# AgentMaker/PAPC

Measured on AMD Instinct MI355X. Metric: point-clouds/sec (fwd+bwd) PointNet++SSG B=32 N=4096, higher is better.
Workload: dtype f32

## Files before the change

### include/papc_hip.h

```cpp
#ifndef PAPC_HIP_H
#define PAPC_HIP_H

#include <stddef.h>
#include <stdint.h>

#ifdef __cplusplus
extern "C" {
#endif

#define PAPC_OK 0
#define PAPC_E_INVALID (-1)
#define PAPC_E_UNSUPPORTED (-2)
#define PAPC_E_LAUNCH (-3)

typedef void *papc_stream_t;

int papc_version(void);
#define PAPC_ABI_VERSION 8
int papc_abi_version(void);
int64_t papc_abi_sizeof(const char *struct_name);
const char *papc_last_error_string(void);


int papc_fps_f32(const float *xyz, int64_t sb, int64_t sn, int64_t sc, int B, int N, int npoint,
// ... 174 lines not shown
int papc_fold_jobs_f32(const papc_fold_job *jobs, int count, papc_stream_t stream);

#define PAPC_SA_MAX_LAYERS 8
#define PAPC_SA_IN_GROUP 0
#define PAPC_SA_IN_ROWS 1
#define PAPC_SA_NO_LINGATHER 1u
#define PAPC_SA_NO_XYZ1 2u
#define PAPC_SA_NO_NOSTORE 4u
#define PAPC_SA_NO_GMAX 8u
#define PAPC_SA_NO_FUSED_RED 16u
#define PAPC_SA_NO_COMPACT 32u
#define PAPC_SA_NO_PLANES 64u
#define PAPC_SA_NO_PLANES_POINTWISE 128u
#define PAPC_SA_NO_XYZ_FUSE 256u
#define PAPC_SA_NO_PSEL 1024u
#define PAPC_SA_NO_GSIGN 2048u
#define PAPC_SA_NO_WSTATS 512u
typedef struct papc_sa_desc {
    int32_t B, N, S, K, D;
    int32_t n_layers;
    int32_t cin;
    int32_t cout[PAPC_SA_MAX_LAYERS];
    int32_t input;
    int32_t identity_rows;
    int32_t xyz_first, pool, eval_bn, cut_gather_grad;
    float eps, momentum;
    uint32_t disable;
    int32_t inference;
    int32_t want_input_grad;
} papc_sa_desc;
typedef struct papc_sa_layer {
    const float *w, *b, *gamma, *beta;
    float *running_mean, *running_var;
} papc_sa_layer;
typedef struct papc_compact_src {
    const int32_t *start, *rows, *cidx, *seg_grp;
    const float *wrow, *coef;
    int32_t G;
} papc_compact_src;
typedef struct papc_sa_io {
    const float *xyz; int64_t sb, sn, sc;
    const float *new_xyz;
    const float *feats;
    const int32_t *idx;
    const float *x_rows;
    const float *xc; const double *xc_gram;
    const papc_compact_src *compact;
    const float *consts3; int32_t consts3_ld;
    papc_sa_layer layer[PAPC_SA_MAX_LAYERS];
    float *out;
    void *saved, *scratch;
    const papc_point_lists *plists;
    const float *wfeat;
} papc_sa_io;
typedef struct papc_sa_plan {
    papc_sa_desc d;
    int32_t cin0;
    int32_t lin0, xyz1, gmax, nostore, compact, sparse_max, planes;
    int64_t saved_bytes, fwd_scratch_bytes, bwd_scratch_bytes;
    int64_t off_y[PAPC_SA_MAX_LAYERS], off_cst[PAPC_SA_MAX_LAYERS], off_argmax;
} papc_sa_plan;
typedef struct papc_sa_grads {
    const float *gout;
    float *dw[PAPC_SA_MAX_LAYERS], *db[PAPC_SA_MAX_LAYERS], *dgamma[PAPC_SA_MAX_LAYERS], *dbeta[PAPC_SA_MAX_LAYERS];
    int32_t acc_w[PAPC_SA_MAX_LAYERS], acc_gb[PAPC_SA_MAX_LAYERS];
    const float *wt[PAPC_SA_MAX_LAYERS];
    float *grad_feats, *grad_x;
    struct papc_fold_list *defer;
} papc_sa_grads;
int papc_sa_mlp_plan(const papc_sa_desc *desc, const papc_sa_io *io, papc_sa_plan *plan);
int papc_sa_mlp_fwd(const papc_sa_plan *plan, const papc_sa_io *io, papc_stream_t stream);
int papc_sa_mlp_bwd(const papc_sa_plan *plan, const papc_sa_io *io, const papc_sa_grads *grads, papc_stream_t stream);

typedef struct papc_pfn_desc {
    int32_t P, T, C;
    float vx, vy, x_offset, y_offset;
    float eps, momentum;
    int32_t training;
    int32_t zero_padded;
} papc_pfn_desc;
typedef struct papc_pfn_io {
    const float *features; const int32_t *num_voxels, *coors;
    const float *w, *gamma, *beta;
    float *running_mean, *running_var;
    float *out;
    void *saved, *scratch;
    uint32_t *tickets;
} papc_pfn_io;
int papc_pfn_workspace(const papc_pfn_desc *desc, int64_t *saved_bytes, int64_t *scratch_bytes);
int papc_pfn_fwd(const papc_pfn_desc *desc, const papc_pfn_io *io, papc_stream_t stream);
int papc_pfn_bwd(const papc_pfn_desc *desc, const papc_pfn_io *io, const float *gout, float *dw, float *dgamma, float *dbeta, int accumulate,
                 papc_stream_t stream);


int papc_pfn_decorate_f32(const float *features, const int32_t *num_voxels, const int32_t *coors, int P, int T,
                          float vx, float vy, float x_offset, float y_offset, int with_distance, float *out,
                          papc_stream_t stream);
int papc_pfn_decorate_nf_f32(const float *features, int F, const int32_t *num_voxels, const int32_t *coors, int P, int T,
                             float vx, float vy, float x_offset, float y_offset, int with_distance, float *out, papc_stream_t stream);
int papc_pfn_stats_f32(const float *features, const int32_t *num_voxels, const int32_t *coors, int P, int T,
                       float vx, float vy, float x_offset, float y_offset, const float *w, int C,
                       float *stats_partial, int *n_blocks_out, papc_stream_t stream);
int papc_pfn_apply_f32(const float *features, const int32_t *num_voxels, const int32_t *coors, int P, int T,
                       float vx, float vy, float x_offset, float y_offset, const float *w, int C,
                       const float *scale, const float *shift, float *out, int32_t *argmax,
                       papc_stream_t stream);
// ... 156 lines not shown
typedef struct papc_pg_prep {
    int mode;
    int64_t M; int C;
    const float *x; int64_t ldx;
    const float *xyz; int64_t sb, sn, sc; const float *feats; int N, D, xyz_first;
    const float *dz;
    const float *gout, *ysel; const int32_t *argmax; int K;
    const float *stats; int parts;
    const float *gamma, *beta; float eps, momentum; float *running_mean, *running_var;
    float *mean, *invstd, *scale, *shift;
    const float *red; int red_parts;
    float *dgamma, *dbeta; int accumulate;
    void *planes, *planes_t;
} papc_pg_prep;
int papc_pg_prep_rows_f32(const papc_pg_prep *args, papc_stream_t stream);

#define PAPC_PG_STORE 0
#define PAPC_PG_FWD 1
#define PAPC_PG_FWD_GMAX 2
#define PAPC_PG_RED 3
typedef struct papc_pg_gemm {
    int epi;
    const void *a, *b;
    int R1, R2, K;
    float *c; int64_t ldc;
    int split; int64_t split_stride;
    const float *bias;
    float *stats;
    float *gmax, *gmin; int32_t *amax, *amin;
    const float *y_prev, *mean, *invstd, *scale, *shift;
    int family;
} papc_pg_gemm;
int papc_pg_gemm_f32(const papc_pg_gemm *args, papc_stream_t stream);
int papc_pg_gemm_group_f32(const papc_pg_gemm *args, int count, papc_stream_t stream);

int papc_pg_final_f32(const float *stats, int parts, int64_t M, int C, const float *gamma, const float *beta, float eps, float momentum,
                      float *mean, float *invstd, float *scale, float *shift, float *running_mean, float *running_var, float *gmax,
                      const float *gmin, const int32_t *amax, const int32_t *amin, int64_t G, float *out, int32_t *argmax, papc_stream_t stream);
int papc_pg_final_groups_f32(const float *stats, int parts, int64_t M, int C, const float *gamma, const float *beta, float eps, float momentum,
                             float *mean, float *invstd, float *scale, float *shift, float *running_mean, float *running_var, const float *gmax,
                             const float *gmin, const int32_t *amax, const int32_t *amin, int64_t G, int tiles_per_group, float *out, int32_t *argmax,
                             float *ysel, papc_stream_t stream);

typedef struct papc_pg_fold_job {
    const float *partial; int nsplit; int64_t stride, n;
    float *out; int accumulate;
} papc_pg_fold_job;
int papc_pg_fold_f32(const papc_pg_fold_job *jobs, int count, papc_stream_t stream);

int papc_transpose_batch_f32(const float *const *src, float *const *dst, const int *rows, const int *cols, int count, papc_stream_t stream);
int papc_transpose_batch_ld_f32(const float *const *src, const int *src_ld, float *const *dst, const int *rows, const int *cols, const int *copy, int count,
                                papc_stream_t stream);

int papc_fill_f32(float *p, int64_t n, float value, papc_stream_t stream);
int papc_copy2d_f32(const float *src, int64_t src_ld, float *dst, int64_t dst_ld, int rows, int cols, int transpose,
                    papc_stream_t stream);
int papc_reduce_partials_strided_f32(const float *partial, int n_chunks, int64_t ld, int rows, int cols, float *out,
                                     int64_t out_ld, int accumulate, papc_stream_t stream);
typedef struct papc_copy_job {
    const float *src;
    float *dst;
    int32_t B, R, C;
    int64_t sb, sr, sc, db, dr, dc;
} papc_copy_job;
int papc_copy_strided_batch_f32(const papc_copy_job *jobs, int count, papc_stream_t stream);
int papc_scale_by_f32(const float *x, const float *scalar, int64_t n, float *out, papc_stream_t stream);

int papc_adam_step_f32(float *param, const float *grad, float *exp_avg, float *exp_avg_sq, int64_t n,
                       float lr, double beta1, double beta2, float eps, float weight_decay, int step,
                       float grad_scale, papc_stream_t stream);
int papc_adam_step_zero_f32(float *param, float *grad, float *exp_avg, float *exp_avg_sq, int64_t n,
                            float lr, double beta1, double beta2, float eps, float weight_decay, int step,
                            float grad_scale, papc_stream_t stream);
int papc_adam_tick(int64_t *step_dev, papc_stream_t stream);
int papc_flag_set(uint32_t *flag, uint32_t value, int64_t *counter, papc_stream_t stream);
int papc_flag_wait(uint32_t *flag, int64_t max_spins, papc_stream_t stream);
int papc_flag_wait_slot(uint32_t *flag, int slot, int64_t max_spins, papc_stream_t stream);
int papc_adam_step_dev_f32(float *param, float *grad, float *exp_avg, float *exp_avg_sq, int64_t n, float lr, double beta1, double beta2,
                           float eps, float weight_decay, const int64_t *step_dev, float grad_scale, int zero_grad, papc_stream_t stream);

#define PAPC_K_FPS 0
#define PAPC_K_BALL_QUERY 1
#define PAPC_K_GROUP 2
#define PAPC_K_MLP_GEMM 3
#define PAPC_K_BN_RELU_MAX 4
#define PAPC_K_BWD_REDUCE 5
#define PAPC_K_BWD_DX 6
#define PAPC_K_BWD_DW 7
#define PAPC_K_PFN 8
#define PAPC_K_MISC 9
#define PAPC_K_COUNT 10
int papc_prof_enable(unsigned mask);
int papc_prof_reset(void);
int papc_prof_read(int kernel, double *total_ms, int64_t *launches);

int papc_knob_set(const char *name, int value);
int papc_knob_get(const char *name, int *value);

#ifdef __cplusplus
}
#endif
#endif
```

### papc_amd/_lib.py

```python
import ctypes
import os

_HERE = os.path.dirname(os.path.abspath(__file__))
LIB_PATH = os.environ.get("PAPC_LIB") or os.path.join(_HERE, "libpapc_hip.so")

ABI_VERSION = 8

c_p = ctypes.c_void_p
c_i = ctypes.c_int
c_l = ctypes.c_int64
c_f = ctypes.c_float


class PapcError(RuntimeError):
    pass


class GroupSrc(ctypes.Structure):
    _fields_ = [("xyz", c_p), ("sb", c_l), ("sn", c_l), ("sc", c_l), ("new_xyz", c_p), ("feats", c_p),
                ("idx", c_p), ("N", c_i), ("S", c_i), ("K", c_i), ("D", c_i), ("xyz_first", c_i),
                ("cidx", c_p), ("seg_grp", c_p), ("rows_dev", c_p), ("wstat", c_p), ("plists", c_p)]


class PointLists(ctypes.Structure):
# ... 93 lines not shown
    "papc_points_to_voxel_f32": (c_i, [c_p, c_i, c_i, c_p, c_p, c_i, c_i, c_i, c_p, c_p, c_p, c_p, c_p, ctypes.c_size_t, c_p]),
    "papc_pillar_scatter_f32": (c_i, [c_p, c_p, c_i, c_i, c_i, c_i, c_i, c_p, c_p, c_p]),
    "papc_pillar_scatter_bwd_f32": (c_i, [c_p, c_p, c_p, c_i, c_i, c_i, c_i, c_i, c_p, c_p]),
    "papc_head_fc_f32": (c_i, [c_p, c_p, c_p, c_p, c_p, c_i, c_i, c_i, c_i, c_f, c_f, c_p, c_p, c_p, c_f, c_p, c_i, c_p, c_p, c_p, c_p,
                               c_p, c_p, c_p]),
    "papc_head_bwd_f32": (c_i, [c_p, c_p, c_i, c_p, c_p, c_p, c_p, c_p, c_f, c_i, c_p, c_i, c_i, c_i, c_p, c_p, c_p, c_p, c_p, c_i, c_p]),
    "papc_softmax_xent_f32": (c_i, [c_p, c_p, c_i, c_i, c_p, c_p, c_p]),
    "papc_head_chain_fwd_f32": (c_i, [c_p, c_i, c_i, c_p, c_p, c_p, c_p, c_p, c_p, c_p]),
    "papc_head_chain_bwd_f32": (c_i, [c_p, c_i, c_i, c_p, c_p]),
    "papc_cloud_transform_f32": (c_i, [c_p, c_l, c_l, c_l, c_p, c_l, c_i, c_i, c_i, c_p, c_p]),
    "papc_cloud_transform_bwd_workspace": (ctypes.c_size_t, [c_i, c_i, c_i]),
    "papc_cloud_transform_bwd_f32": (c_i, [c_p, c_l, c_l, c_l, c_p, c_l, c_p, c_i, c_i, c_i, c_p, c_l, c_l, c_l, c_i, c_p, c_p, ctypes.c_size_t, c_p]),
    "papc_cloud_concat_conv_parts": (c_i, [c_i, c_i]),
    "papc_cloud_concat_conv_f32": (c_i, [c_p, c_l, c_p, c_p, c_p, c_i, c_i, c_i, c_i, c_i, c_p, c_p, c_p, c_p]),
    "papc_cloud_concat_conv_bwd_workspace": (ctypes.c_size_t, [c_i, c_i, c_i, c_i, c_i]),
    "papc_cloud_concat_conv_bwd_f32": (c_i, [c_p, c_p, c_p, c_p, c_p, c_p, c_p, c_p, c_p, c_l, c_p, c_p, c_i, c_i, c_i, c_i, c_i, c_p, c_l, c_i, c_p, c_p,
                                             c_p, c_p, c_p, ctypes.c_size_t, c_p]),
    "papc_nms_workspace": (ctypes.c_size_t, [c_i]),
    "papc_nms_f32": (c_i, [c_p, c_i, c_f, c_p, c_p, c_p, ctypes.c_size_t, c_p]),
    "papc_lingather_parts": (c_i, [c_l]),
    "papc_lingather_fwd_f32": (c_i, [c_p, c_p, c_i, c_p, c_i, c_i, c_p, c_i, c_p, c_p, c_p]),
    "papc_lingather_bwd_f32": (c_i, [c_p, c_p, c_i, c_i, c_p, c_p, c_p]),
    "papc_lingather_bwd_pp_f32": (c_i, [c_p, c_p, c_i, c_i, c_p, c_p, c_i, c_i, c_p, c_p, c_p, c_p]),
    "papc_lingather_list_parts": (c_i, [c_l]),
    "papc_lingather_bwd_parts": (c_i, [c_p, c_i, c_i]),
    "papc_lingather_bwd_lists_ok": (c_i, [c_p, c_i]),
    "papc_point_lists_f32": (c_i, [c_p, c_i, c_p, c_p, c_p, c_p, c_p, c_p]),
    "papc_lingather_bwd_pp_ok": (c_i, [c_p, c_i, c_i]),
    "papc_bn_max_prep_f32": (c_i, [c_p] * 10 + [c_l, c_i, c_i] + [c_p] * 6),
    "papc_mlp_max_nostore_ok": (c_i, [c_l, c_i, c_i, c_i]),
    "papc_mlp_bwd_dw_max_ws_floats": (c_l, [c_l, c_i, c_i]),
    "papc_mlp_bwd_dw_max_f32": (c_i, [c_p, c_p, c_i, c_p, c_p, c_p, c_p, c_p, c_p, c_p, c_l, c_i, c_i, c_p, c_p, c_i, c_p]),
    "papc_mlp_bwd_dx_xyz_ok": (c_i, [c_l, c_i, c_i]),
    "papc_mlp_bwd_dx_xyz_f32": (c_i, [c_p, c_p, c_l, c_i, c_i, c_p, c_p, c_p, c_p]),
    "papc_mlp_bwd_dx_max_f32": (c_i, [c_p, c_p, c_i, c_p, c_l, c_p, c_p, c_p, c_p, c_l, c_i, c_i, c_p, c_p, c_p]),
    "papc_mlp_xyz_ok": (c_i, [c_l, c_i, c_i]),
    "papc_xyz_parts": (c_i, [c_l]),
    "papc_xyz_bwd_parts": (c_i, [c_l]),
    "papc_xyz_group_f32": (c_i, [c_p, c_i, c_p, c_p, c_p]),
    "papc_xyz_gram_fold_f32": (c_i, [c_p, c_i, c_p, c_p]),
    "papc_xyz_l1_finalize_f32": (c_i, [c_p, c_i, c_l, c_p, c_i, c_i, c_p, c_p, c_p, c_f, c_f, c_i] + [c_p] * 9),
    "papc_xyz_l1_bwd_f32": (c_i, [c_p, c_p, c_p, c_l, c_i, c_p, c_p]),
    "papc_xyz_l1_bwd_finalize_f32": (c_i, [c_p, c_i, c_l, c_i, c_p, c_p, c_i, c_i] + [c_p] * 7 + [c_i, c_p]),
    "papc_pg_planes_bytes": (ctypes.c_size_t, [c_l, c_l]),
    "papc_pg_prep_weights_f32": (c_i, [c_p, c_i, c_p]),
    "papc_pg_prep_rows_f32": (c_i, [c_p, c_p]),
    "papc_pg_gemm_f32": (c_i, [c_p, c_p]),
    "papc_pg_gemm_group_f32": (c_i, [c_p, c_i, c_p]),
    "papc_pg_final_f32": (c_i, [c_p, c_i, c_l, c_i, c_p, c_p, c_f, c_f] + [c_p] * 10 + [c_l, c_p, c_p, c_p]),
    "papc_pg_final_groups_f32": (c_i, [c_p, c_i, c_l, c_i, c_p, c_p, c_f, c_f] + [c_p] * 10 + [c_l, c_i, c_p, c_p, c_p, c_p]),
    "papc_pg_fold_f32": (c_i, [c_p, c_i, c_p]),
    "papc_transpose_batch_f32": (c_i, [c_p, c_p, c_p, c_p, c_i, c_p]),
    "papc_transpose_batch_ld_f32": (c_i, [c_p, c_p, c_p, c_p, c_p, c_p, c_i, c_p]),
    "papc_rotate_nms_f32": (c_i, [c_p, c_i, c_f, c_p, c_p, c_p, ctypes.c_size_t, c_p]),
    "papc_rotate_iou_f32": (c_i, [c_p, c_p, c_i, c_i, c_i, c_p, c_p]),
    "papc_rbbox_iou_f32": (c_i, [c_p, c_p, c_p, c_f, c_i, c_i, c_p, c_p]),
    "papc_riou_f32": (c_i, [c_p, c_p, c_f, c_i, c_i, c_p, c_p]),
    "papc_fill_f32": (c_i, [c_p, c_l, c_f, c_p]),
    "papc_copy_strided_batch_f32": (c_i, [c_p, c_i, c_p]),
    "papc_copy2d_f32": (c_i, [c_p, c_l, c_p, c_l, c_i, c_i, c_i, c_p]),
    "papc_reduce_partials_strided_f32": (c_i, [c_p, c_i, c_l, c_i, c_i, c_p, c_l, c_i, c_p]),
    "papc_scale_by_f32": (c_i, [c_p, c_p, c_l, c_p, c_p]),
    "papc_adam_step_f32": (c_i, [c_p, c_p, c_p, c_p, c_l, c_f, ctypes.c_double, ctypes.c_double, c_f, c_f, c_i, c_f, c_p]),
    "papc_adam_step_zero_f32": (c_i, [c_p, c_p, c_p, c_p, c_l, c_f, ctypes.c_double, ctypes.c_double, c_f, c_f, c_i, c_f, c_p]),
    "papc_adam_tick": (c_i, [c_p, c_p]),
    "papc_flag_set": (c_i, [c_p, ctypes.c_uint32, c_p, c_p]),
    "papc_flag_wait": (c_i, [c_p, c_l, c_p]),
    "papc_flag_wait_slot": (c_i, [c_p, c_i, c_l, c_p]),
    "papc_adam_step_dev_f32": (c_i, [c_p, c_p, c_p, c_p, c_l, c_f, ctypes.c_double, ctypes.c_double, c_f, c_f, c_p, c_f, c_i, c_p]),
    "papc_knob_set": (c_i, [ctypes.c_char_p, c_i]),
    "papc_knob_get": (c_i, [ctypes.c_char_p, ctypes.POINTER(c_i)]),
    "papc_prof_enable": (c_i, [ctypes.c_uint]),
    "papc_prof_reset": (c_i, []),
    "papc_prof_read": (c_i, [c_i, ctypes.POINTER(ctypes.c_double), ctypes.POINTER(c_l)]),
}

_lib = None


def load():
    global _lib
    if _lib is None:
        import torch
        if not os.path.exists(LIB_PATH):
            raise PapcError("libpapc_hip.so not found at %s -- build it with `python -m papc_amd.build` "
                            "(there is no CPU fallback)" % LIB_PATH)
        lib = ctypes.CDLL(LIB_PATH)
        missing = [n for n in SIGNATURES if not hasattr(lib, n)]
        if missing:
            raise PapcError("libpapc_hip.so lacks symbols declared in include/papc_hip.h: %s" % ", ".join(missing))
        for name, (res, args) in SIGNATURES.items():
            fn = getattr(lib, name)
            fn.restype = res
            fn.argtypes = args
        if lib.papc_abi_version() != ABI_VERSION:
            raise PapcError("libpapc_hip.so speaks ABI %d, this package ABI %d (include/papc_hip.h: PAPC_ABI_VERSION): rebuild with "
                            "`python -m papc_amd.build`" % (lib.papc_abi_version(), ABI_VERSION))
        _lib = lib
    return _lib


def check(status, what):
    if status != 0:
        msg = load().papc_last_error_string().decode("utf-8", "replace")
        raise PapcError("%s failed (%d): %s" % (what, status, msg))


def stream_ptr():
    import torch
    return torch.cuda.current_stream().cuda_stream


def ptr(t):
    return 0 if t is None else t.data_ptr()


def zeros(shape, device):
    import torch
    t = torch.empty(shape, device=device, dtype=torch.float32)
    if t.numel():
        check(load().papc_fill_f32(t.data_ptr(), t.numel(), 0.0, stream_ptr()), "papc_fill_f32")
    return t


_CONSTS = {}


def _capturing():
    import torch
    return torch.cuda.is_available() and torch.cuda.is_current_stream_capturing()


def const_zeros(shape, device):
    import torch
    key = ("z", tuple(shape), str(device))
    t = _CONSTS.get(key)
    if t is None:
        if _capturing():
            return torch.zeros(tuple(shape), device=device, dtype=torch.float32)
        t = _CONSTS[key] = torch.zeros(tuple(shape), device=device, dtype=torch.float32)
    return t


def const_idx3(B, N, device):
    import torch
    key = ("idx3", str(device))
    rows = int(B) * int(N)
    t = _CONSTS.get(key)
    if t is None or t.shape[0] < rows:
        mk = lambda n: torch.arange(3, device=device, dtype=torch.int32).expand(n, 3).contiguous()
        if _capturing():
            return mk(rows).view(B, N, 3)
        if t is not None:
            _CONSTS.setdefault(("idx3-retired", str(device)), []).append(t)
# ... 17 lines not shown
```

### papc_amd/build.py

```python
import concurrent.futures
import glob
import os
import subprocess
import sys

HERE = os.path.dirname(os.path.abspath(__file__))
ROOT = os.path.dirname(HERE)
CSRC = os.path.join(HERE, "csrc")
OBJ = os.path.join(CSRC, "obj")
LIB = os.path.join(HERE, "libpapc_hip.so")
ARCH = "gfx950"

COMMON = ["--offload-arch=" + ARCH, "-O3", "-std=c++17", "-fPIC", "-fno-fast-math", "-ffp-contract=off",
          "-I", os.path.join(ROOT, "include"), "-I", CSRC, "-Wall", "-Wno-unused-function"]
NOSLP = ["-fno-slp-vectorize"]
RES = ["-Rpass-analysis=kernel-resource-usage"]
EXTRA = {"mlp_stream.hip": NOSLP + RES, "mlp_gemm.hip": NOSLP, "mlp_dw.hip": NOSLP, "sampling.hip": NOSLP, "bn_ops.hip": NOSLP, "folds.hip": NOSLP, "pfn.hip": NOSLP, "interp.hip": NOSLP, "nms.hip": NOSLP, "head.hip": NOSLP, "lingather.hip": NOSLP, "smallm.hip": NOSLP + RES}


def _hipcc():
    for c in (os.environ.get("HIPCC"), "/opt/rocm/bin/hipcc", "hipcc"):
        if c and (os.path.isabs(c) and os.path.exists(c) or not os.path.isabs(c)):
            return c
    return "hipcc"


def _check_no_spills(remarks):
    import re
    name = None
    seen = set()
    for line in remarks.splitlines():
        m = re.search(r"Function Name: (\S+)", line)
        if m:
            name = m.group(1)
        m = re.search(r"(VGPRs Spill|SGPRs Spill|ScratchSize \[bytes/lane\]): (\d+)", line)
        if m and name and "stream_kernel" in name and "Lb1E" in name:
            seen.add(name)
            if int(m.group(2)) != 0 and "SGPRs Spill" not in m.group(1):
                raise RuntimeError("mlp_stream.hip: %s has %s = %s (asm-loaded registers must not spill)" % (name, m.group(1), m.group(2)))
    if not seen:
        raise RuntimeError("mlp_stream.hip: no kernel-resource-usage remark of an asm-ring stream_kernel was found; the spill guard cannot vouch for this build")


def _audit_asm_ring(asm_path):
    from ._isa_audit import audit, report
    res = audit(open(asm_path).read(), "stream_kernel")
    if res["violations"] or not res["kernels"] or res["loads"] == 0:
        raise RuntimeError("mlp_stream.hip: the asm-ring audit failed (%d kernels, %d hidden loads scanned)\n%s"
                           % (len(res["kernels"]), res["loads"], report(res)[-2000:]))


def _audit_pfn_tickets(cmd):
    from ._isa_audit import audit_ticket
    asm = os.path.join(OBJ, "pfn.s")
    cmd_s = list(cmd)
    cmd_s[cmd_s.index("-c")] = "-S"
    cmd_s[cmd_s.index("-o") + 1] = asm
    r2 = subprocess.run(cmd_s + ["--cuda-device-only"], stdout=subprocess.PIPE, stderr=subprocess.STDOUT, text=True)
    if r2.returncode != 0:
        raise RuntimeError("hipcc -S failed on pfn.hip\n" + r2.stdout[-2000:])
    res = audit_ticket(open(asm).read())
    os.remove(asm)
    if res["violations"] or res["atomics"] == 0:
        raise RuntimeError("pfn.hip: the ticket audit failed (%d ticket atomics scanned): %s" % (res["atomics"], res["violations"][:4]))


def _newest(paths):
    return max(os.path.getmtime(p) for p in paths)


# ... 57 lines not shown
```

### papc_amd/csrc/bn_ops.hip

```cpp
#include "common.h"

namespace papc {

template <int V> struct Vec;
template <> struct Vec<4> {
    float4 v;
    __device__ static Vec load(const float *p) { Vec r; r.v = *reinterpret_cast<const float4 *>(p); return r; }
    __device__ void store(float *p) const { *reinterpret_cast<float4 *>(p) = v; }
    __device__ float &operator[](int i) { return (&v.x)[i]; }
    __device__ float operator[](int i) const { return (&v.x)[i]; }
};
template <> struct Vec<1> {
    float v;
    __device__ static Vec load(const float *p) { Vec r; r.v = *p; return r; }
    __device__ void store(float *p) const { *p = v; }
    __device__ float &operator[](int) { return v; }
    __device__ float operator[](int) const { return v; }
};

template <int D>
__device__ __forceinline__ void sum_partial_rows_d(const float *__restrict__ part, int n_tiles, int C, int c, int tl, double &s1, double &s2)
{
    for (int t0 = tl; t0 < n_tiles; t0 += 64 * D) {
        float a[D], b[D];
#pragma unroll
        for (int j = 0; j < D; ++j) {
            const int t = t0 + 64 * j;
            const int64_t o = (int64_t)(t < n_tiles ? t : t0) * 2 * C + c;
            a[j] = part[o];
            b[j] = part[o + C];
        }
#pragma unroll
        for (int j = 0; j < D; ++j) {
            if (t0 + 64 * j < n_tiles) { s1 += (double)a[j]; s2 += (double)b[j]; }
        }
    }
}
__device__ __forceinline__ void sum_partial_rows(const float *__restrict__ part, int n_tiles, int C, int c, int tl, double &s1, double &s2)
{
    if (n_tiles > 512) sum_partial_rows_d<16>(part, n_tiles, C, c, tl, s1, s2);
    else sum_partial_rows_d<8>(part, n_tiles, C, c, tl, s1, s2);
}

__device__ __forceinline__ double lane_get(double v, int l)
{
    const int lo = __builtin_amdgcn_readlane(__double2loint(v), l), hi = __builtin_amdgcn_readlane(__double2hiint(v), l);
    return __hiloint2double(hi, lo);
}
__device__ __forceinline__ void fold_part_lanes(double &s1, double &s2)
{
    s1 += __shfl_xor(s1, 1); s2 += __shfl_xor(s2, 1);
    s1 += __shfl_xor(s1, 2); s2 += __shfl_xor(s2, 2);
    double t1 = 0.0, t2 = 0.0;
// ... 402 lines not shown
        if (cc < C) {
            out[g * C + cc] = b;
            if (argmax) argmax[g * C + cc] = bk;
        }
    }
}

__global__ __launch_bounds__(256) void bn_max_psel_kernel(const float *__restrict__ gout, const float *__restrict__ ysel,
                                                          const float *__restrict__ scale, const float *__restrict__ shift, int64_t total,
                                                          int C, float *__restrict__ psel)
{
    for (int64_t e = (int64_t)blockIdx.x * blockDim.x + threadIdx.x; e < total; e += (int64_t)gridDim.x * blockDim.x) {
        const int c = (int)(e % C);
        const float sc = scale[c];
        psel[e] = fmaf(sc, ysel[e], shift[c]) > 0.f ? sc * gout[e] : 0.f;
    }
}

__global__ __launch_bounds__(256) void bn_max_wcat_kernel(const float *__restrict__ w, const float *__restrict__ bias,
                                                          const float *__restrict__ scale, const float *__restrict__ mean,
                                                          const float *__restrict__ invstd, const float *__restrict__ c1,
                                                          const float *__restrict__ c2, int Co, int Ci, float *__restrict__ wcat,
                                                          float *__restrict__ hbias, float *__restrict__ e_out, float *__restrict__ q_out)
{
    extern __shared__ float sm[];
    float *ewn = sm;
    double *red = reinterpret_cast<double *>(sm + ((Co + 1) & ~1));
    const int n = blockIdx.x, tid = threadIdx.x;
    double hacc = 0.0;
    for (int c = tid; c < Co; c += 256) {
        const float s = scale[c];
        const float e = s * c2[c] * invstd[c];
        const float q = e * (mean[c] - (bias ? bias[c] : 0.f)) - s * c1[c];
        const float wv = w[(int64_t)c * Ci + n];
        ewn[c] = e * wv;
        hacc += (double)q * (double)wv;
        wcat[(int64_t)n * (Co + Ci) + c] = wv;
        if (n == 0) { e_out[c] = e; q_out[c] = q; }
    }
    red[tid] = hacc;
    __syncthreads();
    for (int st = 128; st > 0; st >>= 1) {
        if (tid < st) red[tid] += red[tid + st];
        __syncthreads();
    }
    if (tid == 0) hbias[n] = (float)red[0];
    for (int j = tid; j < Ci; j += 256) {
        double g = 0.0;
        for (int c = 0; c < Co; ++c) g += (double)ewn[c] * (double)w[(int64_t)c * Ci + j];
        wcat[(int64_t)n * (Co + Ci) + Co + j] = (float)(-g);
    }
}

struct TransposeBatch {
    const float *src[8];
    float *dst[8];
    int rows[8], cols[8];
    int ld[8], copy[8];
};

__global__ __launch_bounds__(256) void transpose_batch_kernel(TransposeBatch t)
{
    __shared__ float tile[32][33];
    const int m = blockIdx.y;
    const int rows = t.rows[m], cols = t.cols[m];
    const int tiles_c = (cols + 31) >> 5, tiles = ((rows + 31) >> 5) * tiles_c;
    const float *__restrict__ src = t.src[m];
    float *__restrict__ dst = t.dst[m];
    const int tx = threadIdx.x & 31, ty = threadIdx.x >> 5;
    for (int tl = blockIdx.x; tl < tiles; tl += gridDim.x) {
        const int r0 = (tl / tiles_c) * 32, c0 = (tl % tiles_c) * 32;
#pragma unroll
        for (int i = 0; i < 4; ++i) {
            const int r = r0 + ty + 8 * i, c = c0 + tx;
            const float v = (r < rows && c < cols) ? src[(int64_t)r * t.ld[m] + c] : 0.f;
            tile[ty + 8 * i][tx] = v;
            if (t.copy[m] && r < rows && c < cols) dst[(int64_t)r * cols + c] = v;
        }
        if (t.copy[m]) continue;
        __syncthreads();
#pragma unroll
        for (int i = 0; i < 4; ++i) {
            const int c = c0 + ty + 8 * i, r = r0 + tx;
            if (r < rows && c < cols) dst[(int64_t)c * rows + r] = tile[tx][ty + 8 * i];
        }
        __syncthreads();
    }
}

}


using namespace papc;

extern "C" {

int papc_bn_finalize_f32(const float *stats_partial, int n_tiles, int64_t M, int C, const float *gamma,
                         const float *beta, float eps, float momentum, float *mean, float *invstd,
                         float *scale, float *shift, float *running_mean, float *running_var,
                         papc_stream_t stream)
{
    PAPC_REQUIRE(stats_partial && mean && invstd && scale && shift, PAPC_E_INVALID, "papc_bn_finalize_f32: null pointer");
    PAPC_REQUIRE(n_tiles >= 1 && M >= 1 && C >= 1, PAPC_E_INVALID, "papc_bn_finalize_f32: bad sizes");
    hipStream_t st = as_stream(stream);
    ProfScope prof(PAPC_K_MISC, st);
    hipLaunchKernelGGL(bn_finalize_kernel, dim3((unsigned)C), dim3(64), 0, st, stats_partial, n_tiles, M, C, gamma,
                       beta, eps, momentum, mean, invstd, scale, shift, running_mean, running_var);
    return check_launch("papc_bn_finalize_f32");
}

int papc_bn_relu_max_f32(const float *y, const float *scale, const float *shift, int64_t G, int K, int C,
                         float *out, int32_t *argmax, papc_stream_t stream)
{
    PAPC_REQUIRE(y && scale && shift && out, PAPC_E_INVALID, "papc_bn_relu_max_f32: null pointer");
    PAPC_REQUIRE(G >= 1 && K >= 1 && C >= 1, PAPC_E_INVALID, "papc_bn_relu_max_f32: bad sizes");
    hipStream_t st = as_stream(stream);
    ProfScope prof(PAPC_K_BN_RELU_MAX, st);
    const bool v4 = (C % 4 == 0) && aligned16(y) && aligned16(scale) && aligned16(shift) && aligned16(out);
    if (v4 && K >= 256 && G * (C / 4) < 65536 && G <= 65535) {
        hipLaunchKernelGGL(bn_relu_max_split_kernel, dim3((unsigned)G, (unsigned)cdiv(C, 256)), dim3(1024), 0, st, y, scale, shift, G, K, C, out, argmax);
        return check_launch("papc_bn_relu_max_f32");
    }
    if (v4) hipLaunchKernelGGL(bn_relu_max_kernel<4>, dim3(ew_grid(G * (C / 4))), dim3(256), 0, st, y, scale, shift, G, K, C, out, argmax);
    else hipLaunchKernelGGL(bn_relu_max_kernel<1>, dim3(ew_grid(G * C)), dim3(256), 0, st, y, scale, shift, G, K, C, out, argmax);
    return check_launch("papc_bn_relu_max_f32");
}

int papc_bn_select_max_f32(float *gmax, const float *gmin, const int32_t *amax, const int32_t *amin,
                           const float *scale, const float *shift, int64_t G, int C, float *out, int32_t *argmax,
                           papc_stream_t stream)
{
    PAPC_REQUIRE(gmax && gmin && amax && amin && scale && shift && out, PAPC_E_INVALID, "papc_bn_select_max_f32: null pointer");
    PAPC_REQUIRE(G >= 1 && C >= 1, PAPC_E_INVALID, "papc_bn_select_max_f32: bad sizes");
    hipStream_t st = as_stream(stream);
    ProfScope prof(PAPC_K_BN_RELU_MAX, st);
    hipLaunchKernelGGL(bn_select_max_kernel, dim3(ew_grid(G * C)), dim3(256), 0, st, gmax, gmin, amax, amin, scale, shift, G * C, C, out, argmax);
    return check_launch("papc_bn_select_max_f32");
}

int papc_bn_relu_f32(const float *y, const float *scale, const float *shift, int64_t M, int C, float *z, papc_stream_t stream)
// ... 256 lines not shown
```

### papc_amd/csrc/capi.hip

```cpp
#include <stdarg.h>
#include <string.h>

#include <mutex>
#include <vector>

#include "common.h"

#define GEMM_PARTS_DEFAULT 768

namespace papc {

static thread_local char g_err[512] = "";

void set_error(const char *fmt, ...)
{
    va_list ap;
    va_start(ap, fmt);
    vsnprintf(g_err, sizeof(g_err), fmt, ap);
    va_end(ap);
}

int check_launch(const char *what)
{
    hipError_t e = hipGetLastError();
    if (e != hipSuccess) {
        set_error("%s: %s", what, hipGetErrorString(e));
        return PAPC_E_LAUNCH;
    }
    return PAPC_OK;
}

struct KnobDef { const char *name; int def, lo, hi; };
static const KnobDef g_knob_defs[KNOB_COUNT] = {
    {"PAPC_LG_PARTS", 2048, 1, 8192},
    {"PAPC_DW_F32", 0, 0, 1},
    {"PAPC_DW_DBG", 0, 0, 1},
    {"PAPC_DW_XYZ", 1, 0, 1},
    {"PAPC_PARTS", GEMM_PARTS_DEFAULT, 1, 1024},
    {"PAPC_GEMM_F32", 0, 0, 1},
    {"PAPC_GEMM_WAVES", 0, 0, 8},
    {"PAPC_MAXCAT_WAVES", 8, 4, 8},
    {"PAPC_GEMM_WS", 0, 0, 3},
    {"PAPC_GEMM_OCC", 0, 0, 1},
    {"PAPC_GEMM_DBG", 0, 0, 1},
    {"PAPC_GEMM_KB", 0, 0, 2},
    {"PAPC_GEMM_MINWG", 192, 1, 4096},
    {"PAPC_GEMM_TL", 0, 0, 1},
    {"PAPC_FPS_THREADS", 0, 0, 1024},
    {"PAPC_FPS_THREADS_SMALL", 0, 0, 1024},
    {"PAPC_STREAM", 1, 0, 1},
    {"PAPC_STREAM_MINTILES", 2048, 1, 1 << 30},
    {"PAPC_STREAM_CK", 0, 0, 8},
    {"PAPC_STREAM_ASM", 1, 0, 1},
    {"PAPC_PFN_MFMA", 1, 0, 1},
    {"PAPC_DW_RS64", 1, 0, 1},
    {"PAPC_DW_ROWS", 1, 0, 1},
    {"PAPC_DW_ROWS_BLOCKS", 4, 1, 16},
    {"PAPC_DW_ROWSX", 1, 0, 1},
    {"PAPC_PG_DBG", 0, 0, 15},
    {"PAPC_PG_NB", 0, 0, 2},
    {"PAPC_PG_NS", 0, 0, 3},
    {"PAPC_STREAM_MAXCAT", 1, 0, 1},
    {"PAPC_MAX_NOSTORE", 1, 0, 1},
    {"PAPC_PFN_FUSED_TAILS", 1, 0, 1},
    {"PAPC_STREAM_NW12", 1, 0, 1},
    {"PAPC_LG_LISTS", 1, 0, 1},
    {"PAPC_FOLD_WAVES", 16, 8, 16},
    {"PAPC_LGL_VARIANT", 0, 0, 3},
    {"PAPC_LG_PP", 1, 0, 1},
    {"PAPC_PG_GROUP", 1, 0, 1},
};
static int g_knobs[KNOB_COUNT];
static int knob_parse(int id, const char *e)
{
    const KnobDef &d = g_knob_defs[id];
    if (!e || !*e) return d.def;
    const int v = atoi(e);
    return (v < d.lo || v > d.hi) ? d.def : v;
}
static const bool g_knobs_loaded = [] {
    for (int i = 0; i < KNOB_COUNT; ++i) g_knobs[i] = knob_parse(i, getenv(g_knob_defs[i].name));
    return true;
}();
int knob(int id) { return g_knobs[id]; }

struct ProfState {
    std::mutex mu;
    unsigned mask = 0;
    std::vector<std::pair<hipEvent_t, hipEvent_t>> pending[PAPC_K_COUNT];
    std::vector<hipEvent_t> pool;
    double total_ms[PAPC_K_COUNT] = {0};
    int64_t launches[PAPC_K_COUNT] = {0};
};
static ProfState g_prof;

static hipEvent_t prof_get_event()
{
    if (!g_prof.pool.empty()) {
        hipEvent_t e = g_prof.pool.back();
        g_prof.pool.pop_back();
        return e;
    }
    hipEvent_t e;
    if (hipEventCreate(&e) != hipSuccess) return nullptr;
    return e;
}

ProfScope::ProfScope(int k, hipStream_t s) : kernel(k), stream(s), on(false), e0(nullptr)
{
    if (!(g_prof.mask & (1u << k))) return;
    std::lock_guard<std::mutex> lk(g_prof.mu);
    e0 = prof_get_event();
    if (!e0) return;
    on = hipEventRecord(e0, stream) == hipSuccess;
}

ProfScope::~ProfScope()
{
    if (!on) return;
    std::lock_guard<std::mutex> lk(g_prof.mu);
    hipEvent_t e1 = prof_get_event();
    if (!e1) return;
    if (hipEventRecord(e1, stream) == hipSuccess) g_prof.pending[kernel].push_back({e0, e1});
}

static void prof_drain(int k)
{
    for (auto &pr : g_prof.pending[k]) {
        float ms = 0.f;
        if (hipEventSynchronize(pr.second) == hipSuccess && hipEventElapsedTime(&ms, pr.first, pr.second) == hipSuccess) {
            g_prof.total_ms[k] += ms;
            g_prof.launches[k] += 1;
        }
        g_prof.pool.push_back(pr.first);
        g_prof.pool.push_back(pr.second);
    }
    g_prof.pending[k].clear();
}

}

extern "C" {

int papc_version(void) { return 600;  }

int papc_abi_version(void) { return PAPC_ABI_VERSION; }

int64_t papc_abi_sizeof(const char *struct_name)
{
    if (!struct_name) return -1;
#define PAPC_SIZEOF(T) if (strcmp(struct_name, #T) == 0) return (int64_t)sizeof(T);
    PAPC_SIZEOF(papc_group_src)
    PAPC_SIZEOF(papc_point_lists)
    PAPC_SIZEOF(papc_group_max)
    PAPC_SIZEOF(papc_bwd_dy)
    PAPC_SIZEOF(papc_scatter_dst)
    PAPC_SIZEOF(papc_bwd_red)
    PAPC_SIZEOF(papc_reduce_job)
    PAPC_SIZEOF(papc_fold_job)
    PAPC_SIZEOF(papc_fold_list)
    PAPC_SIZEOF(papc_sa_desc)
    PAPC_SIZEOF(papc_sa_layer)
    PAPC_SIZEOF(papc_compact_src)
    PAPC_SIZEOF(papc_sa_io)
    PAPC_SIZEOF(papc_sa_plan)
    PAPC_SIZEOF(papc_sa_grads)
    PAPC_SIZEOF(papc_pfn_desc)
    PAPC_SIZEOF(papc_pfn_io)
    PAPC_SIZEOF(papc_head_fc_layer)
    PAPC_SIZEOF(papc_head_bwd_job)
    PAPC_SIZEOF(papc_pg_wjob)
    PAPC_SIZEOF(papc_pg_prep)
    PAPC_SIZEOF(papc_pg_gemm)
    PAPC_SIZEOF(papc_pg_fold_job)
    PAPC_SIZEOF(papc_copy_job)
#undef PAPC_SIZEOF
    return -1;
}

const char *papc_last_error_string(void) { return papc::g_err; }

int papc_knob_set(const char *name, int value)
{
    PAPC_REQUIRE(name, PAPC_E_INVALID, "papc_knob_set: null name");
    for (int i = 0; i < papc::KNOB_COUNT; ++i)
        if (!strcmp(name, papc::g_knob_defs[i].name)) {
            PAPC_REQUIRE(value >= papc::g_knob_defs[i].lo && value <= papc::g_knob_defs[i].hi, PAPC_E_INVALID,
                         "papc_knob_set: %s = %d outside [%d, %d]", name, value, papc::g_knob_defs[i].lo, papc::g_knob_defs[i].hi);
            papc::g_knobs[i] = value;
            return PAPC_OK;
        }
    papc::set_error("papc_knob_set: unknown knob %s", name);
    return PAPC_E_INVALID;
}

int papc_knob_get(const char *name, int *value)
{
    PAPC_REQUIRE(name && value, PAPC_E_INVALID, "papc_knob_get: null argument");
    for (int i = 0; i < papc::KNOB_COUNT; ++i)
        if (!strcmp(name, papc::g_knob_defs[i].name)) { *value = papc::g_knobs[i]; return PAPC_OK; }
    papc::set_error("papc_knob_get: unknown knob %s", name);
    return PAPC_E_INVALID;
}

int papc_prof_enable(unsigned mask)
{
    std::lock_guard<std::mutex> lk(papc::g_prof.mu);
    papc::g_prof.mask = mask;
    return PAPC_OK;
}

int papc_prof_reset(void)
{
    std::lock_guard<std::mutex> lk(papc::g_prof.mu);
    for (int k = 0; k < PAPC_K_COUNT; ++k) {
        papc::prof_drain(k);
        papc::g_prof.total_ms[k] = 0;
        papc::g_prof.launches[k] = 0;
    }
    return PAPC_OK;
}

int papc_prof_read(int kernel, double *total_ms, int64_t *launches)
{
    PAPC_REQUIRE(kernel >= 0 && kernel < PAPC_K_COUNT, PAPC_E_INVALID, "papc_prof_read: bad kernel id %d", kernel);
    std::lock_guard<std::mutex> lk(papc::g_prof.mu);
    papc::prof_drain(kernel);
    if (total_ms) *total_ms = papc::g_prof.total_ms[kernel];
// ... 6 lines not shown
```

### papc_amd/csrc/common.h

```cpp
#pragma once
#include <hip/hip_runtime.h>
#include <stdint.h>
#include <stdio.h>
#include <stdlib.h>
#include <string.h>
#include <algorithm>

#include "papc_hip.h"

namespace papc {

void set_error(const char *fmt, ...);
int check_launch(const char *what);

#define PAPC_REQUIRE(cond, code, ...)      \
    do {                                   \
        if (!(cond)) {                     \
            papc::set_error(__VA_ARGS__);  \
            return (code);                 \
        }                                  \
    } while (0)

enum Knob {
    KNOB_LG_PARTS, KNOB_DW_F32, KNOB_DW_DBG, KNOB_DW_XYZ, KNOB_PARTS, KNOB_GEMM_F32, KNOB_GEMM_WAVES, KNOB_MAXCAT_WAVES,
    KNOB_GEMM_WS, KNOB_GEMM_OCC, KNOB_GEMM_DBG, KNOB_GEMM_KB, KNOB_GEMM_MINWG, KNOB_GEMM_TL, KNOB_FPS_THREADS,
    KNOB_FPS_THREADS_SMALL, KNOB_STREAM, KNOB_STREAM_MINTILES, KNOB_STREAM_CK, KNOB_STREAM_ASM, KNOB_PFN_MFMA, KNOB_DW_RS64, KNOB_DW_ROWS, KNOB_DW_ROWS_BLOCKS, KNOB_DW_ROWSX, KNOB_PG_DBG, KNOB_PG_NB, KNOB_PG_NS, KNOB_STREAM_MAXCAT, KNOB_MAX_NOSTORE, KNOB_PFN_FUSED_TAILS, KNOB_STREAM_NW12, KNOB_LG_LISTS, KNOB_FOLD_WAVES, KNOB_LGL_VARIANT, KNOB_LG_PP, KNOB_PG_GROUP, KNOB_COUNT
};
int knob(int id);

struct ProfScope {
    int kernel;
    hipStream_t stream;
    bool on;
    hipEvent_t e0;
    ProfScope(int kernel, hipStream_t stream);
    ~ProfScope();
};

static inline hipStream_t as_stream(papc_stream_t s) { return reinterpret_cast<hipStream_t>(s); }

static inline int64_t cdiv(int64_t a, int64_t b) { return (a + b - 1) / b; }
static inline bool aligned16(const void *p) { return (reinterpret_cast<uintptr_t>(p) & 15) == 0; }

#define PAPC_DPP(v, ctrl, rmask) __builtin_amdgcn_update_dpp((int)(v), (int)(v), (ctrl), (rmask), 0xF, false)

__device__ __forceinline__ float wave_sum_f32_to_lane63(float v)
{
    float t;
    t = __int_as_float(PAPC_DPP(__float_as_int(v), 0xB1, 0xF));  v += t;
    t = __int_as_float(PAPC_DPP(__float_as_int(v), 0x4E, 0xF));  v += t;
    t = __int_as_float(PAPC_DPP(__float_as_int(v), 0x124, 0xF)); v += t;
    t = __int_as_float(PAPC_DPP(__float_as_int(v), 0x128, 0xF)); v += t;
    t = __int_as_float(__builtin_amdgcn_update_dpp(0, __float_as_int(v), 0x142, 0xA, 0xF, false)); v += t;
    t = __int_as_float(__builtin_amdgcn_update_dpp(0, __float_as_int(v), 0x143, 0xC, 0xF, false)); v += t;
    return v;
}

__device__ __forceinline__ float half_sum_f32(float v)
{
    float t;
    t = __int_as_float(PAPC_DPP(__float_as_int(v), 0xB1, 0xF));  v += t;
    t = __int_as_float(PAPC_DPP(__float_as_int(v), 0x4E, 0xF));  v += t;
    t = __int_as_float(PAPC_DPP(__float_as_int(v), 0x124, 0xF)); v += t;
    t = __int_as_float(PAPC_DPP(__float_as_int(v), 0x128, 0xF)); v += t;
    t = __int_as_float(__builtin_amdgcn_update_dpp(0, __float_as_int(v), 0x142, 0xA, 0xF, false)); v += t;
    return v;
}

__device__ __forceinline__ float readlane63_f32(float v)
{
    return __int_as_float(__builtin_amdgcn_readlane(__float_as_int(v), 63));
}


#define PAPC_DPPF(v, ctrl, rmask) __int_as_float(__builtin_amdgcn_update_dpp(__float_as_int(v), __float_as_int(v), (ctrl), (rmask), 0xF, false))
#define PAPC_DPPU(v, ctrl, rmask) ((unsigned)__builtin_amdgcn_update_dpp((int)(v), (int)(v), (ctrl), (rmask), 0xF, false))

__device__ __forceinline__ float row_max_f32(float v)
{
    v = fmaxf(v, PAPC_DPPF(v, 0xB1, 0xF));
    v = fmaxf(v, PAPC_DPPF(v, 0x4E, 0xF));
// ... 75 lines not shown
```

### papc_amd/csrc/sa_mlp.hip

```cpp
#include "common.h"

#define SA_CALL(expr)                 \
    do {                              \
        const int rc__ = (expr);      \
        if (rc__ != PAPC_OK) return rc__; \
    } while (0)

namespace papc {
int pfn_gram_stats(const float *features, const int32_t *num_voxels, const int32_t *coors, int P, int T, float vx, float vy, float x_offset, float y_offset, int zero_padded,
                   double *gram_partial, const float *w, int C, const float *gamma, const float *beta, float eps, float momentum, float *mean, float *invstd,
                   float *scale, float *shift, float *running_mean, float *running_var, double *gram, unsigned *ticket, hipStream_t st);
int pfn_gram_impl(const float *features, const int32_t *num_voxels, const int32_t *coors, int P, int T, float vx, float vy, float x_offset, float y_offset,
                  double *gram_partial, int zero_padded, papc_stream_t stream);
int pfn_apply_impl(const float *features, const int32_t *num_voxels, const int32_t *coors, int P, int T, float vx, float vy, float x_offset, float y_offset,
                   const float *w, int C, const float *scale, const float *shift, float *out, int32_t *argmax, int zero_padded, papc_stream_t stream);
int pfn_bwd_sparse_impl(const float *features, const int32_t *num_voxels, const int32_t *coors, int P, int T, float vx, float vy, float x_offset, float y_offset,
                        const float *w, int C, const float *gout, const int32_t *argmax, const float *mean, const float *invstd, const float *scale,
                        const float *shift, float *partial, int zero_padded, papc_stream_t stream);
int pfn_bwd_fold_finalize(const float *partial, int n_chunks, float *sums, int64_t M, const float *w, int C, const double *gram, const float *mean,
                          const float *invstd, const float *scale, float *dgamma, float *dbeta, float *dw, int flags, unsigned *ticket, hipStream_t st);

constexpr int A_PLAIN_ = PAPC_A_PLAIN, A_BNRELU_ = PAPC_A_BNRELU, A_GROUP_ = PAPC_A_GROUP, A_XYZ_ = PAPC_A_XYZ;

struct Carver {
// ... 192 lines not shown
        s.argmax = c.take<int32_t>((size_t)T * p.d.cout[L - 1]);
        s.gbuf_f = c.take<float>(2 * (size_t)T * p.d.cout[L - 1]);
        s.ysel = p.d.K > PG_GROUP ? c.take<float>((size_t)(M / p.d.K) * p.d.cout[L - 1]) : s.gbuf_f;
    }
    if (!p.d.inference)
        for (int l = 0; l < L; ++l) {
            s.PT[l] = c.take<char>(papc_pg_planes_bytes(cin_of(p, l), M));
            if (l > 0) s.wtp[l] = c.take<char>(papc_pg_planes_bytes(cin_of(p, l), p.d.cout[l]));
            else if (p.d.want_input_grad) s.wtp[0] = c.take<char>(papc_pg_planes_bytes(pg_n_in(p), p.d.cout[0]));
        }
    return c.off;
}

static size_t layout_planes_fwd(const papc_sa_plan &p, void *base, PlanesFwd &f)
{
    Carver c{reinterpret_cast<char *>(base), 0};
    const int L = p.d.n_layers;
    const int64_t M = rows_of(p.d), T = M / PG_GROUP;
    memset(&f, 0, sizeof(f));
    size_t pmax = papc_pg_planes_bytes(M, p.cin0);
    for (int l = 0; l < L; ++l) {
        f.wp[l] = c.take<char>(papc_pg_planes_bytes(p.d.cout[l], cin_of(p, l)));
        f.stats[l] = c.take<float>((size_t)T * 2 * p.d.cout[l]);
        if (l < L - 1) pmax = std::max(pmax, papc_pg_planes_bytes(M, p.d.cout[l]));
    }
    f.P = c.take<char>(pmax);
    if (p.d.pool) f.gbuf_i = c.take<int32_t>(2 * (size_t)T * p.d.cout[L - 1]);
    return c.off;
}

static size_t layout_planes_bwd(const papc_sa_plan &p, void *base, PlanesBwd &b)
{
    Carver c{reinterpret_cast<char *>(base), 0};
    const int L = p.d.n_layers;
    const int64_t M = rows_of(p.d), T = M / PG_GROUP;
    memset(&b, 0, sizeof(b));
    int cmax = p.cin0;
    size_t pm = 0, pmt = 0;
    for (int l = 0; l < L; ++l) {
        cmax = std::max(cmax, p.d.cout[l]);
        pm = std::max(pm, papc_pg_planes_bytes(M, p.d.cout[l]));
        pmt = std::max(pmt, papc_pg_planes_bytes(p.d.cout[l], M));
        b.part[l] = c.take<float>((size_t)pg_split_for(p.d.cout[l], cin_of(p, l), (int)(M / 32)) * p.d.cout[l] * cin_of(p, l));
    }
    b.dyp = c.take<char>(pm);
    b.dypt = c.take<char>(pmt);
    b.dz[0] = c.take<float>((size_t)M * cmax);
    b.dz[1] = c.take<float>((size_t)M * cmax);
    for (int i = 0; i < 3; ++i) b.red[i] = c.take<float>((size_t)T * 2 * cmax);
    b.tmp_gb = c.take<float>(2 * (size_t)cmax);
    return c.off;
}

static int planes_fwd(const papc_sa_plan &p, const papc_sa_io &io, papc_stream_t st)
{
    const papc_sa_desc &d = p.d;
    const int L = d.n_layers;
    const int64_t M = rows_of(d), T = M / PG_GROUP;
    const bool plain = d.input == PAPC_SA_IN_ROWS, want_bwd = !d.inference;
    PlanesSaved s; PlanesFwd f;
    layout_planes_saved(p, io.saved, s);
    layout_planes_fwd(p, io.scratch, f);
    {
        papc_pg_wjob jobs[2 * PAPC_SA_MAX_LAYERS];
        int n = 0;
        const int fcol0 = plain ? 0 : (d.xyz_first ? 3 : 0);
        for (int l = 0; l < L; ++l) {
            const int cin = cin_of(p, l), cout = d.cout[l];
            jobs[n++] = papc_pg_wjob{io.layer[l].w, cin, 1, cout, cin, f.wp[l]};
            if (s.wtp[l]) {
                if (l > 0) jobs[n++] = papc_pg_wjob{io.layer[l].w, 1, cin, cin, cout, s.wtp[l]};
                else jobs[n++] = papc_pg_wjob{io.layer[l].w + fcol0, 1, cin, pg_n_in(p), cout, s.wtp[l]};
            }
        }
        for (int j0 = 0; j0 < n; j0 += 8) SA_CALL(papc_pg_prep_weights_f32(jobs + j0, std::min(8, n - j0), st));
    }
    papc_pg_prep a;
    memset(&a, 0, sizeof(a));
    a.M = M; a.C = p.cin0; a.planes = f.P; a.planes_t = want_bwd ? s.PT[0] : nullptr;
    if (plain) { a.mode = PAPC_PG_PLAIN; a.x = io.x_rows; a.ldx = p.cin0; }
    else { a.mode = PAPC_PG_CONCAT; a.xyz = io.xyz; a.sb = io.sb; a.sn = io.sn; a.sc = io.sc; a.feats = io.feats; a.N = d.N; a.D = d.D; a.xyz_first = d.xyz_first; }
    SA_CALL(papc_pg_prep_rows_f32(&a, st));
    for (int l = 0; l < L; ++l) {
        const papc_sa_layer &ly = io.layer[l];
        const int cout = d.cout[l], cin = cin_of(p, l);
        float *cst = s.cst[l];
        const bool last_pool = l == L - 1 && d.pool;
        papc_pg_gemm g;
        memset(&g, 0, sizeof(g));
        g.epi = last_pool ? PAPC_PG_FWD_GMAX : PAPC_PG_FWD;
        g.a = f.P; g.b = f.wp[l]; g.R1 = (int)M; g.R2 = cout; g.K = cin;
        g.c = s.y[l]; g.ldc = cout; g.split = 1; g.bias = ly.b; g.stats = f.stats[l]; g.family = PAPC_K_MLP_GEMM;
        if (last_pool) { g.gmax = s.gbuf_f; g.gmin = s.gbuf_f + T * cout; g.amax = f.gbuf_i; g.amin = f.gbuf_i + T * cout; }
        SA_CALL(papc_pg_gemm_f32(&g, st));
        if (l < L - 1) {
            papc_pg_prep b;
            memset(&b, 0, sizeof(b));
            b.mode = PAPC_PG_BNRELU; b.M = M; b.C = cout; b.x = s.y[l]; b.ldx = cout; b.stats = f.stats[l]; b.parts = (int)T;
            b.gamma = ly.gamma; b.beta = ly.beta; b.eps = d.eps; b.momentum = d.momentum; b.running_mean = ly.running_mean; b.running_var = ly.running_var;
            b.mean = cst; b.invstd = cst + cout; b.scale = cst + 2 * cout; b.shift = cst + 3 * cout;
            b.planes = f.P; b.planes_t = want_bwd ? s.PT[l + 1] : nullptr;
            SA_CALL(papc_pg_prep_rows_f32(&b, st));
        } else if (!d.pool) {
            SA_CALL(papc_bn_finalize_f32(f.stats[l], (int)T, M, cout, ly.gamma, ly.beta, d.eps, d.momentum, cst, cst + cout, cst + 2 * cout, cst + 3 * cout,
                                         ly.running_mean, ly.running_var, st));
            SA_CALL(papc_bn_relu_f32(s.y[l], cst + 2 * cout, cst + 3 * cout, M, cout, io.out, st));
        } else if (d.K > PG_GROUP) {
            SA_CALL(papc_pg_final_groups_f32(f.stats[l], (int)T, M, cout, ly.gamma, ly.beta, d.eps, d.momentum, cst, cst + cout, cst + 2 * cout, cst + 3 * cout,
                                             ly.running_mean, ly.running_var, s.gbuf_f, s.gbuf_f + T * cout, f.gbuf_i, f.gbuf_i + T * cout, M / d.K, d.K / PG_GROUP,
                                             io.out, s.argmax, s.ysel, st));
        } else {
            SA_CALL(papc_pg_final_f32(f.stats[l], (int)T, M, cout, ly.gamma, ly.beta, d.eps, d.momentum, cst, cst + cout, cst + 2 * cout, cst + 3 * cout,
                                      ly.running_mean, ly.running_var, s.gbuf_f, s.gbuf_f + T * cout, f.gbuf_i, f.gbuf_i + T * cout, T, io.out, s.argmax, st));
        }
    }
    return PAPC_OK;
}

static int planes_bwd(const papc_sa_plan &p, const papc_sa_io &io, const papc_sa_grads &gr, papc_stream_t st)
{
    const papc_sa_desc &d = p.d;
    const int L = d.n_layers;
    const int64_t M = rows_of(d), T = M / PG_GROUP;
    const bool plain = d.input == PAPC_SA_IN_ROWS;
    PAPC_REQUIRE(!d.inference, PAPC_E_INVALID, "papc_sa_mlp_bwd: the forward ran with desc.inference set");
    PlanesSaved s; PlanesBwd b;
    layout_planes_saved(p, io.saved, s);
    layout_planes_bwd(p, io.scratch, b);
    int cmaxc = 0;
    for (int l = 0; l < L; ++l) cmaxc = std::max(cmaxc, d.cout[l]);
    float *grad_in = plain ? gr.grad_x : gr.grad_feats;
    PAPC_REQUIRE(!grad_in || s.wtp[0], PAPC_E_INVALID, "papc_sa_mlp_bwd: an input gradient needs desc.want_input_grad at the forward");
    papc_pg_fold_job fold[PAPC_SA_MAX_LAYERS];
    int n_fold = 0;
    const float *dz = nullptr, *red = nullptr;
    int flip = 0;
    for (int l = L - 1; l >= 0; --l) {
        const int cout = d.cout[l], cin = cin_of(p, l);
        const float *cst = s.cst[l];
        const bool acc_w = gr.acc_w[l] != 0, acc_gb = gr.acc_gb[l] != 0;
        float *dgamma = gr.dgamma[l] ? gr.dgamma[l] : b.tmp_gb, *dbeta = gr.dbeta[l] ? gr.dbeta[l] : b.tmp_gb + cmaxc;
        PAPC_REQUIRE(gr.dw[l], PAPC_E_INVALID, "papc_sa_mlp_bwd: dw[%d] is NULL", l);
        const bool need_dx = l > 0 || grad_in;
        papc_pg_prep a;
        memset(&a, 0, sizeof(a));
        a.M = M; a.C = cout; a.x = s.y[l]; a.ldx = cout; a.mean = const_cast<float *>(cst); a.invstd = const_cast<float *>(cst + cout);
        a.scale = const_cast<float *>(cst + 2 * cout); a.shift = const_cast<float *>(cst + 3 * cout);
        a.dgamma = dgamma; a.dbeta = dbeta; a.accumulate = (acc_gb && gr.dgamma[l]) ? 1 : 0; a.planes = need_dx ? b.dyp : nullptr; a.planes_t = b.dypt;
        if (l == L - 1 && !d.pool) {
            SA_CALL(papc_bn_bwd_reduce_f32(PAPC_DZ_DENSE, gr.gout, nullptr, nullptr, 1, s.y[l], cst, cst + cout, cst + 2 * cout, cst + 3 * cout, M, cout, (int)T, b.red[2], st));
            a.mode = PAPC_PG_DY_DENSE; a.dz = gr.gout; a.red = b.red[2]; a.red_parts = (int)T;
        } else if (l == L - 1) {
            a.mode = PAPC_PG_DY_MAX; a.gout = gr.gout; a.ysel = s.ysel; a.argmax = s.argmax; a.K = d.K;
        } else {
            a.mode = PAPC_PG_DY_DENSE; a.dz = dz; a.red = red; a.red_parts = (int)T;
        }
        SA_CALL(papc_pg_prep_rows_f32(&a, st));
        papc_pg_gemm g[2];
        memset(g, 0, sizeof(g));
        int ng = 0;
        float *dz_prev = nullptr, *red_prev = nullptr;
        if (l > 0) {
            const float *pc = s.cst[l - 1];
            dz_prev = b.dz[flip]; red_prev = b.red[flip];
            flip ^= 1;
            papc_pg_gemm &x = g[ng++];
            x.epi = PAPC_PG_RED; x.a = b.dyp; x.b = s.wtp[l]; x.R1 = (int)M; x.R2 = cin; x.K = cout;
            x.c = dz_prev; x.ldc = cin; x.split = 1; x.stats = red_prev; x.family = PAPC_K_BWD_DX;
            x.y_prev = s.y[l - 1]; x.mean = pc; x.invstd = pc + cin; x.scale = pc + 2 * cin; x.shift = pc + 3 * cin;
        } else if (grad_in) {
            const int n_in = pg_n_in(p);
            papc_pg_gemm &x = g[ng++];
            x.epi = PAPC_PG_STORE; x.a = b.dyp; x.b = s.wtp[0]; x.R1 = (int)M; x.R2 = n_in; x.K = cout;
            x.c = grad_in; x.ldc = n_in; x.split = 1; x.family = PAPC_K_BWD_DX;
        }
        const int split = pg_split_for(cout, cin, (int)(M / 32));
        papc_pg_gemm &w = g[ng++];
        w.epi = PAPC_PG_STORE; w.a = b.dypt; w.b = s.PT[l]; w.R1 = cout; w.R2 = cin; w.K = (int)M;
        w.c = b.part[l]; w.ldc = cin; w.split = split; w.split_stride = (int64_t)cout * cin; w.family = PAPC_K_BWD_DW;
        SA_CALL(papc_pg_gemm_group_f32(g, ng, st));
        if (!defer_fold(gr, b.part[l], split, (int64_t)cout * cin, 1, cout * cin, gr.dw[l], (int64_t)cout * cin, acc_w ? 1 : 0))
// ... 57 lines not shown
            plan->off_y[l] = l < L ? (int64_t)(reinterpret_cast<char *>(ps.y[l]) - fake) : -1;
            plan->off_cst[l] = l < L ? (int64_t)(reinterpret_cast<char *>(ps.cst[l]) - fake) : -1;
        }
        plan->off_argmax = ps.argmax ? (int64_t)(reinterpret_cast<char *>(ps.argmax) - fake) : -1;
        plan->saved_bytes = (int64_t)layout_planes_saved(*plan, nullptr, ps) + 256;
        plan->fwd_scratch_bytes = (int64_t)layout_planes_fwd(*plan, nullptr, pf) + 256;
        plan->bwd_scratch_bytes = (int64_t)layout_planes_bwd(*plan, nullptr, pb) + 256;
        return PAPC_OK;
    }
    plan->lin0 = !(d.disable & PAPC_SA_NO_LINGATHER) && !ev && !plain && has_idx && has_feats && L >= 2 && d.D % 4 == 0 && d.D >= 16 &&
                 d.cout[0] % 4 == 0 && d.cout[0] <= 256;
    plan->xyz1 = !(d.disable & PAPC_SA_NO_XYZ1) && !ev && !plain && has_idx && !has_feats && d.D == 0 && L >= 3 &&
                 papc_mlp_xyz_ok(M, d.cout[0], d.cout[1]);
    plan->compact = plan->lin0 && d.pool && !(d.disable & PAPC_SA_NO_COMPACT) && io && io->compact && papc_mlp_compact_ok(M, d.K, L, d.cout);
    const int cL = d.cout[L - 1], cLi = L > 1 ? d.cout[L - 2] : plan->cin0;
    plan->gmax = !plan->compact && d.pool && !(d.disable & PAPC_SA_NO_GMAX) && !ev && papc_mlp_gemm_gmax_ok(M, cL, d.K);
    plan->nostore = plan->gmax && !(d.disable & PAPC_SA_NO_NOSTORE) && L >= 2 && !(L == 2 && plan->xyz1) && papc_mlp_max_nostore_ok(M, cLi, cL, d.K);
    plan->sparse_max = plan->nostore;
    SavedPtrs s; FwdPtrs f; BwdPtrs b;
    {
        char *fake = reinterpret_cast<char *>((uintptr_t)1 << 40);
        layout_saved(*plan, fake, s);
        for (int l = 0; l < PAPC_SA_MAX_LAYERS; ++l) {
            plan->off_y[l] = (l < L && s.y[l]) ? (int64_t)(reinterpret_cast<char *>(s.y[l]) - fake) : -1;
            plan->off_cst[l] = (l < L && s.cst[l]) ? (int64_t)(reinterpret_cast<char *>(s.cst[l]) - fake) : -1;
        }
        plan->off_argmax = s.argmax ? (int64_t)(reinterpret_cast<char *>(s.argmax) - fake) : -1;
    }
    plan->saved_bytes = (int64_t)layout_saved(*plan, nullptr, s) + 256;
    plan->fwd_scratch_bytes = (int64_t)layout_fwd(*plan, nullptr, f) + 256;
    plan->bwd_scratch_bytes = (int64_t)layout_bwd(*plan, nullptr, b) + 256;
    return PAPC_OK;
}

int papc_sa_mlp_fwd(const papc_sa_plan *plan, const papc_sa_io *io, papc_stream_t st)
{
    PAPC_REQUIRE(plan && io && io->out && io->saved && io->scratch, PAPC_E_INVALID, "papc_sa_mlp_fwd: null pointer");
    const papc_sa_plan &p = *plan;
    const papc_sa_desc &d = p.d;
    const int L = d.n_layers;
    const int64_t M = rows_of(d), G = (int64_t)d.B * d.S;
    const bool plain = d.input == PAPC_SA_IN_ROWS, ev = d.eval_bn != 0;
    PAPC_REQUIRE(plain ? io->x_rows != nullptr : (io->xyz && io->new_xyz), PAPC_E_INVALID, "papc_sa_mlp_fwd: missing input");
    PAPC_REQUIRE(plain || d.identity_rows || io->idx, PAPC_E_INVALID, "papc_sa_mlp_fwd: grouped input without idx (set identity_rows for sample_and_group_all)");
    PAPC_REQUIRE(plain || d.D == 0 || io->feats, PAPC_E_INVALID, "papc_sa_mlp_fwd: D = %d but feats is NULL", d.D);
    PAPC_REQUIRE(!p.compact || io->compact, PAPC_E_INVALID, "papc_sa_mlp_fwd: the plan is compacted but io->compact is NULL");
    if (p.planes) {
        for (int l = 0; l < L; ++l) PAPC_REQUIRE(io->layer[l].w && io->layer[l].gamma && io->layer[l].beta, PAPC_E_INVALID, "papc_sa_mlp_fwd: layer %d lacks w / gamma / beta", l);
        return planes_fwd(p, *io, st);
    }
    SavedPtrs s; FwdPtrs f;
    layout_saved(p, io->saved, s);
    layout_fwd(p, io->scratch, f);
    const int parts = papc_mlp_gemm_parts(M);
    const bool wstats = p.compact && !(d.disable & PAPC_SA_NO_WSTATS);
    const int R_c = (p.compact && !wstats) ? papc_compact_corr_parts() : 0;
    papc_group_src grp;
    if (!plain) fill_grp(grp, d, *io, p.compact);
    if (!plain && wstats) grp.wstat = io->compact->wrow;
    int cmax = 0;
    for (int l = 0; l < L; ++l) cmax = std::max(cmax, d.cout[l]);
    const size_t stats_stride = (size_t)(std::max(parts, p.lin0 ? papc_lingather_parts(M) : 0) + R_c) * 2 * cmax;

    const float *prev_y = nullptr, *prev_sc = nullptr, *prev_sh = nullptr;
    int cin = p.cin0;
    const float *xc = nullptr;
    papc_group_max gm;
    memset(&gm, 0, sizeof(gm));
    for (int l = 0; l < L; ++l) {
        const papc_sa_layer &ly = io->layer[l];
        PAPC_REQUIRE(ly.w && ly.gamma && ly.beta, PAPC_E_INVALID, "papc_sa_mlp_fwd: layer %d lacks w / gamma / beta", l);
        PAPC_REQUIRE(!ev || (ly.running_mean && ly.running_var), PAPC_E_INVALID, "papc_sa_mlp_fwd: eval_bn needs the running statistics");
        const int cout = d.cout[l];
        float *stats = ev ? nullptr : f.stats + (size_t)l * stats_stride;
        int parts_l = parts;
        const papc_group_max *gm_ref = nullptr;
        if (l == L - 1 && p.gmax) {
            gm.gmax = s.gbuf_f; gm.gmin = s.gbuf_f + G * cout; gm.amax = f.gbuf_i; gm.amin = f.gbuf_i + G * cout; gm.K = d.K;
            gm.sign_src = (d.disable & PAPC_SA_NO_GSIGN) ? nullptr : ly.gamma;
            gm_ref = &gm;
        }
        float *y = s.y[l];
        float *cst = s.cst[l];
        if (l == 0 && p.xyz1) {
            const double *gpart1;
            if (io->xc && io->xc_gram) { xc = io->xc; gpart1 = io->xc_gram; }
            else {
                SA_CALL(papc_xyz_group_f32(&grp, d.B, s.xc, f.gpart + 16, st));
                SA_CALL(papc_xyz_gram_fold_f32(f.gpart + 16, papc_xyz_parts(M), f.gpart, st));
                xc = s.xc; gpart1 = f.gpart;
            }
            SA_CALL(papc_xyz_l1_finalize_f32(gpart1, 1, M, ly.w, cin, 0, ly.b, ly.gamma, ly.beta, d.eps, d.momentum, cout, cst, cst + cout, cst + 2 * cout,
                                             cst + 3 * cout, ly.running_mean, ly.running_var, s.wf, s.gram, st));
            prev_y = nullptr; prev_sc = cst + 2 * cout; prev_sh = cst + 3 * cout;
            cin = cout;
            continue;
        }
        if (l == 1 && p.xyz1) {
            SA_CALL(papc_mlp_gemm_f32(A_XYZ_, xc, 4, nullptr, s.wf, nullptr, ly.w, ly.b, M, cin, cout, y, stats, gm_ref, st));
        } else if (l == 0 && plain) {
            SA_CALL(papc_mlp_gemm_f32(A_PLAIN_, io->x_rows, cin, nullptr, nullptr, nullptr, ly.w, ly.b, M, cin, cout, y, stats, gm_ref, st));
        } else if (l == 0 && p.lin0) {
            const int fcol0 = d.xyz_first ? 3 : 0;
            const float *wfeat = io->wfeat;
            if (!wfeat) {
                SA_CALL(papc_copy2d_f32(ly.w + fcol0, cin, f.wfeat, d.D, cout, d.D, 0, st));
                wfeat = f.wfeat;
            }
            const int64_t BN = (int64_t)d.B * d.N;
            SA_CALL(papc_mlp_gemm_f32(A_PLAIN_, io->feats, d.D, nullptr, nullptr, nullptr, wfeat, nullptr, BN, d.D, cout, s.P, nullptr, nullptr, st));
            parts_l = papc_lingather_parts(M);
            SA_CALL(papc_lingather_fwd_f32(s.P, &grp, d.B, ly.w, cin, d.xyz_first ? 0 : d.D, ly.b, cout, y, stats, st));
        } else if (l == 0) {
            SA_CALL(papc_mlp_gemm_f32(A_GROUP_, nullptr, 0, &grp, nullptr, nullptr, ly.w, ly.b, M, cin, cout, y, stats, gm_ref, st));
        } else if (p.compact) {
            SA_CALL(papc_mlp_gemm_rows_w_f32(A_BNRELU_, prev_y, cin, nullptr, prev_sc, prev_sh, ly.w, ly.b, M, cin, cout, y, stats, nullptr, io->compact->rows,
                                             wstats ? io->compact->wrow : nullptr, st));
        } else {
            SA_CALL(papc_mlp_gemm_f32(A_BNRELU_, prev_y, cin, nullptr, prev_sc, prev_sh, ly.w, ly.b, M, cin, cout, y, stats, gm_ref, st));
        }
        if (p.compact && !wstats) {
            SA_CALL(papc_bn_stats_corr_f32(y, cout, io->compact->start, io->compact->coef, io->compact->G, stats + (size_t)parts_l * 2 * cout, st));
            parts_l += R_c;
        }
        if (ev) SA_CALL(papc_bn_eval_consts_f32(ly.running_mean, ly.running_var, ly.gamma, ly.beta, d.eps, cout, cst, cst + cout, cst + 2 * cout, cst + 3 * cout, st));
        else SA_CALL(papc_bn_finalize_f32(stats, parts_l, M, cout, ly.gamma, ly.beta, d.eps, d.momentum, cst, cst + cout, cst + 2 * cout, cst + 3 * cout,
                                          ly.running_mean, ly.running_var, st));
        prev_y = y; prev_sc = cst + 2 * cout; prev_sh = cst + 3 * cout;
        cin = cout;
    }
    if (!d.pool) return papc_bn_relu_f32(prev_y, prev_sc, prev_sh, M, cin, io->out, st);
    if (p.compact) return papc_bn_relu_max_seg_f32(prev_y, cin, io->compact->start, prev_sc, prev_sh, (int)G, io->out, s.argmax, s.gbuf_f, st);
    if (p.gmax) return papc_bn_select_max_f32(s.gbuf_f, s.gbuf_f + G * cin, f.gbuf_i, f.gbuf_i + G * cin, prev_sc, prev_sh, G, cin, io->out, s.argmax, st);
    return papc_bn_relu_max_f32(prev_y, prev_sc, prev_sh, G, d.K, cin, io->out, s.argmax, st);
}

int papc_sa_mlp_bwd(const papc_sa_plan *plan, const papc_sa_io *io, const papc_sa_grads *gr, papc_stream_t st)
{
    PAPC_REQUIRE(plan && io && gr && gr->gout && io->saved && io->scratch, PAPC_E_INVALID, "papc_sa_mlp_bwd: null pointer");
    const papc_sa_plan &p = *plan;
    const papc_sa_desc &d = p.d;
    const int L = d.n_layers;
    const int64_t M = rows_of(d), G = (int64_t)d.B * d.S;
    const bool plain = d.input == PAPC_SA_IN_ROWS, ev = d.eval_bn != 0;
    if (p.planes) return planes_bwd(p, *io, *gr, st);
    SavedPtrs s; BwdPtrs b;
    layout_saved(p, io->saved, s);
    layout_bwd(p, io->scratch, b);
    const float *xc = p.xyz1 ? ((io->xc && io->xc_gram) ? io->xc : s.xc) : nullptr;
    papc_group_src grp;
    if (!plain) fill_grp(grp, d, *io, p.compact);
    const int n_parts = (int)std::min<int64_t>(512, (M + 127) / 128);
    const int gemm_parts = papc_mlp_gemm_parts(M);
    const bool x_needs = plain && gr->grad_x, f_needs = !plain && d.D > 0 && gr->grad_feats && !d.cut_gather_grad;
    const float *ysel = (p.gmax || p.compact) ? s.gbuf_f : nullptr;
    const float *ones = io->consts3, *zeros = nullptr, *big = nullptr;
    int cmaxc = 0;
    for (int l = 0; l < L; ++l) cmaxc = std::max(cmaxc, d.cout[l]);
    if (p.lin0) {
        PAPC_REQUIRE(io->consts3 && io->consts3_ld >= d.cout[0], PAPC_E_INVALID, "papc_sa_mlp_bwd: the gather-add first layer needs consts3 (ones | zeros | 1e30 rows of >= %d floats)", d.cout[0]);
        zeros = io->consts3 + io->consts3_ld; big = io->consts3 + 2 * (int64_t)io->consts3_ld;
    }

    bool need_wt[PAPC_SA_MAX_LAYERS];
    const float *wts[PAPC_SA_MAX_LAYERS];
    for (int l = 0; l < L; ++l) {
        need_wt[l] = l > 0 || x_needs || f_needs;
        wts[l] = nullptr;
    }
    if (p.sparse_max) need_wt[L - 1] = false;
    if (p.lin0) need_wt[0] = false;
    {
        const float *srcs[8]; float *dsts[8]; int rws[8], cls[8];
        int n = 0;
        for (int l = 0; l < L; ++l) {
            if (!need_wt[l]) continue;
            if (gr->wt[l]) { wts[l] = gr->wt[l]; continue; }
            srcs[n] = io->layer[l].w; dsts[n] = b.wt[l]; rws[n] = d.cout[l]; cls[n] = cin_of(p, l);
            wts[l] = b.wt[l];
            if (++n == 8) { SA_CALL(papc_transpose_batch_f32(srcs, dsts, rws, cls, n, st)); n = 0; }
        }
        if (n) SA_CALL(papc_transpose_batch_f32(srcs, dsts, rws, cls, n, st));
    }

    papc_reduce_job jobs[PAPC_SA_MAX_LAYERS];
    int n_jobs = 0;
    bool xyz_fused = false;
    bool dz0_masked = false;
    const float *dz = nullptr;
    const float *fused_red = nullptr;
    int flip = 0;
    for (int l = L - 1; l >= 0; --l) {
        const papc_sa_layer &ly = io->layer[l];
        const int cout = d.cout[l], cin = cin_of(p, l);
        const float *cst = s.cst[l];
        float *c12 = b.c12[l];
        const bool acc_w = gr->acc_w[l] != 0, acc_gb = gr->acc_gb[l] != 0 && !ev;
        float *dgamma = gr->dgamma[l] ? gr->dgamma[l] : b.tmp_gb, *dbeta = gr->dbeta[l] ? gr->dbeta[l] : b.tmp_gb + cmaxc;
        PAPC_REQUIRE(gr->dw[l], PAPC_E_INVALID, "papc_sa_mlp_bwd: dw[%d] is NULL", l);
        papc_bwd_dy dy;
        memset(&dy, 0, sizeof(dy));
// ... 217 lines not shown
```

### papc_amd/csrc/smallm.hip

```cpp
#include "fold.h"
#include "mlp_loaders.h"

namespace papc {

enum { PG_EPI_STORE = 0, PG_EPI_FWD = 1, PG_EPI_FWD_GMAX = 2, PG_EPI_RED = 3 };
enum { PG_PREP_PLAIN = 0, PG_PREP_CONCAT = 1, PG_PREP_BNRELU = 2, PG_PREP_DY_DENSE = 3, PG_PREP_DY_MAX = 4 };

__host__ __device__ static inline int64_t ru64(int64_t a, int64_t b) { return (a + b - 1) / b * b; }

__device__ __forceinline__ void store_planes8(char *frag0, int slot, const float (&v)[8])
{
    bf16x8 pl[3];
    split8(v, pl);
    *reinterpret_cast<uint4 *>(frag0 + slot * 16) = __builtin_bit_cast(uint4, pl[0]);
    *reinterpret_cast<uint4 *>(frag0 + 1024 + slot * 16) = __builtin_bit_cast(uint4, pl[1]);
    *reinterpret_cast<uint4 *>(frag0 + 2048 + slot * 16) = __builtin_bit_cast(uint4, pl[2]);
}

struct WJob {
    const float *src; int64_t sr, sc;
    int R, K;
    char *dst;
};
struct WJobs {
    WJob j[8];
};

__global__ __launch_bounds__(256) void pg_prep_w_kernel(WJobs jobs)
{
    const WJob jb = jobs.j[blockIdx.y];
    const int KB = (int)(ru64(jb.K, 32) / 16), RB = (int)(ru64(jb.R, 32) / 32);
    const int lane = threadIdx.x & 63, wv = threadIdx.x >> 6;
    const int r_in = lane & 31, h = lane >> 5;
    for (int f = blockIdx.x * 4 + wv; f < RB * KB; f += gridDim.x * 4) {
        const int rb = f / KB, kb = f - rb * KB;
        const int r = rb * 32 + r_in, k0 = kb * 16 + h * 8;
        float v[8];
#pragma unroll
        for (int i = 0; i < 8; ++i) v[i] = (r < jb.R && k0 + i < jb.K) ? jb.src[(int64_t)r * jb.sr + (int64_t)(k0 + i) * jb.sc] : 0.f;
        store_planes8(jb.dst + ((int64_t)rb * KB + kb) * 3072, lane, v);
    }
}

struct PrepArgs {
    int64_t M; int C;
    const float *x; int64_t ldx;
    const float *xyz; int64_t sb, sn, sc; const float *feats; int N, D, xyz_first;
    const float *dz;
    const float *gout, *ysel; const int32_t *argmax; int K;
    const float *stats; int parts;
    const float *gamma, *beta; float eps, momentum; float *rmean, *rvar;
    float *mean, *invstd, *scale, *shift;
    const float *red; int red_parts;
    float *dgamma, *dbeta; int accumulate;
    char *P; int KBp;
    char *PT; int KBt;
};

template <int MODE>
__device__ __forceinline__ void prep_consts(const PrepArgs &p, int cb, float (*cs)[32], double (*rd)[8][32])
{
    const int cl = threadIdx.x & 31, pl = threadIdx.x >> 5;
    const int c = cb * 32 + cl;
    const bool cok = c < p.C;
    double s1 = 0.0, s2 = 0.0;
    if (MODE == PG_PREP_BNRELU) {
        if (cok) for (int t = pl; t < p.parts; t += 8) { s1 += (double)p.stats[(int64_t)t * 2 * p.C + c]; s2 += (double)p.stats[((int64_t)t * 2 + 1) * p.C + c]; }
    } else if (p.red) {
        if (cok) for (int t = pl; t < p.red_parts; t += 8) { s1 += (double)p.red[(int64_t)t * 2 * p.C + c]; s2 += (double)p.red[((int64_t)t * 2 + 1) * p.C + c]; }
    } else if (MODE == PG_PREP_DY_MAX) {
        if (cok) {
            const float sc = p.scale[c], sh = p.shift[c], mu = p.mean[c], is = p.invstd[c];
            const int64_t G = p.M / p.K;
            for (int64_t g = pl; g < G; g += 8) {
                const float yv = p.ysel[g * p.C + c];
                const float pv = fmaf(sc, yv, sh) > 0.f ? p.gout[g * p.C + c] : 0.f;
                s1 += (double)pv;
                s2 += (double)(pv * ((yv - mu) * is));
            }
        }
    }
    rd[0][pl][cl] = s1; rd[1][pl][cl] = s2;
    __syncthreads();
    if (threadIdx.x < 32) {
        s1 = 0.0; s2 = 0.0;
#pragma unroll
        for (int q = 0; q < 8; ++q) { s1 += rd[0][q][cl]; s2 += rd[1][q][cl]; }
        const bool first = blockIdx.y == 0;
        if (MODE == PG_PREP_BNRELU) {
            float sc = 0.f, sh = 0.f;
            if (cok) {
                const double mu = s1 / (double)p.M;
                double var = s2 / (double)p.M - mu * mu;
                if (var < 0.0) var = 0.0;
// ... 696 lines not shown
```

### papc_amd/csrc/xyz1.hip

```cpp
#include "mlp_loaders.h"

namespace papc {

constexpr int XYZ_T = 256;
constexpr int XYZ_MAX_PARTS = 512;

__global__ __launch_bounds__(XYZ_T) void xyz_group_kernel(GroupSrc g, int64_t M, float4 *__restrict__ xc, double *__restrict__ partial)
{
    __shared__ double red[XYZ_T / 64][10];
    double s[10];
#pragma unroll
    for (int i = 0; i < 10; ++i) s[i] = 0.0;
    const int64_t per = (M + gridDim.x - 1) / gridDim.x;
    const int64_t m0 = (int64_t)blockIdx.x * per, m1 = min(M, m0 + per);
    for (int64_t m = m0 + threadIdx.x; m < m1; m += XYZ_T) {
        const uint32_t grp = fdiv((uint32_t)m, g.divK);
        const uint32_t b = fdiv(grp, g.divS);
        int j = g.idx ? g.idx[m] : (int)(m - (int64_t)b * g.S * g.K);
        const bool ok = j >= 0 && j < g.N;
        j = ok ? j : 0;
        const float *pp = g.xyz + (int64_t)b * g.sb + (int64_t)j * g.sn;
        const float *qq = g.new_xyz + (int64_t)grp * 3;
        float x = pp[0] - qq[0], y = pp[g.sc] - qq[1], z = pp[2 * g.sc] - qq[2];
        if (!ok) { x = 0.f; y = 0.f; z = 0.f; }
        xc[m] = make_float4(x, y, z, 0.f);
        const double dx = x, dy = y, dz = z;
        s[0] += dx; s[1] += dy; s[2] += dz;
        s[3] += dx * dx; s[4] += dx * dy; s[5] += dx * dz; s[6] += dy * dy; s[7] += dy * dz; s[8] += dz * dz;
        s[9] += 1.0;
    }
    const int lane = threadIdx.x & 63, wave = threadIdx.x >> 6;
#pragma unroll
    for (int i = 0; i < 10; ++i) {
        double v = s[i];
#pragma unroll
        for (int o = 32; o >= 1; o >>= 1) v += __shfl_xor(v, o);
        if (lane == 0) red[wave][i] = v;
    }
    __syncthreads();
    if (threadIdx.x < 10) {
        double v = 0.0;
#pragma unroll
        for (int w = 0; w < XYZ_T / 64; ++w) v += red[w][threadIdx.x];
        partial[(int64_t)blockIdx.x * 16 + threadIdx.x] = v;
    }
}

__global__ __launch_bounds__(256) void xyz_gram_fold_kernel(const double *__restrict__ partial, int parts, double *__restrict__ gram)
{
    __shared__ double red[16][16];
    const int e = threadIdx.x & 15, sl = threadIdx.x >> 4;
    double s = 0.0;
    if (e < 10) for (int t = sl; t < parts; t += 16) s += partial[(int64_t)t * 16 + e];
    red[sl][e] = s;
    __syncthreads();
    if (threadIdx.x < 16) {
        double v = 0.0;
#pragma unroll
        for (int q = 0; q < 16; ++q) v += red[q][threadIdx.x];
        gram[threadIdx.x] = threadIdx.x < 10 ? v : 0.0;
    }
}

__global__ __launch_bounds__(256) void xyz_l1_finalize_kernel(const double *__restrict__ partial, int parts, double M, const float *__restrict__ w, int ldw,
                                                              int xcol0, const float *__restrict__ bias, const float *__restrict__ gamma,
                                                              const float *__restrict__ beta, float eps, float momentum, int C, float *mean,
                                                              float *invstd, float *scale, float *shift, float *rmean, float *rvar, float *wf,
                                                              double *gram)
{
    __shared__ double red[16][16];
    __shared__ double G[10];
    const int e = threadIdx.x & 15, sl = threadIdx.x >> 4;
    double s = 0.0;
    if (e < 10) for (int t = sl; t < parts; t += 16) s += partial[(int64_t)t * 16 + e];
    red[sl][e] = s;
    __syncthreads();
    if (threadIdx.x < 10) {
        double v = 0.0;
#pragma unroll
        for (int q = 0; q < 16; ++q) v += red[q][threadIdx.x];
        G[threadIdx.x] = v;
        gram[threadIdx.x] = v;
    }
    __syncthreads();
    for (int c = threadIdx.x; c < C; c += 256) {
        const double w0 = w[(int64_t)c * ldw + xcol0], w1 = w[(int64_t)c * ldw + xcol0 + 1], w2 = w[(int64_t)c * ldw + xcol0 + 2];
        const double b = bias ? (double)bias[c] : 0.0;
        const double mx = G[0] / M, my = G[1] / M, mz = G[2] / M;
        const double cxx = G[3] / M - mx * mx, cxy = G[4] / M - mx * my, cxz = G[5] / M - mx * mz;
        const double cyy = G[6] / M - my * my, cyz = G[7] / M - my * mz, czz = G[8] / M - mz * mz;
        const double mu = w0 * mx + w1 * my + w2 * mz + b;
        double var = w0 * (w0 * cxx + w1 * cxy + w2 * cxz) + w1 * (w0 * cxy + w1 * cyy + w2 * cyz) + w2 * (w0 * cxz + w1 * cyz + w2 * czz);
        if (var < 0.0) var = 0.0;
        const double is = 1.0 / sqrt(var + (double)eps);
        const double sc = (gamma ? (double)gamma[c] : 1.0) * is;
        const double sh = (beta ? (double)beta[c] : 0.0) - mu * sc;
        mean[c] = (float)mu; invstd[c] = (float)is; scale[c] = (float)sc; shift[c] = (float)sh;
        if (rmean) rmean[c] = momentum * rmean[c] + (1.f - momentum) * (float)mu;
        if (rvar) rvar[c] = momentum * rvar[c] + (1.f - momentum) * (float)var;
        wf[c * 4 + 0] = (float)(sc * w0); wf[c * 4 + 1] = (float)(sc * w1); wf[c * 4 + 2] = (float)(sc * w2);
        wf[c * 4 + 3] = (float)(sc * b + sh);
    }
}

__global__ __launch_bounds__(XYZ_T) void xyz_l1_bwd_kernel(const float *__restrict__ dz, const float4 *__restrict__ xc, const float *__restrict__ wf,
                                                           int64_t M, int C, int64_t rows_per_chunk, float *__restrict__ partial)
{
    __shared__ float red[XYZ_T * 16];
    const int tid = threadIdx.x;
    const int CQ = C >> 2;
    const int RSL = XYZ_T / CQ;
    const int cq = tid % CQ, slot = tid / CQ;
    const bool act = slot < RSL;
    const int c = cq * 4;
    float4 k[4];
#pragma unroll
    for (int i = 0; i < 4; ++i) k[i] = ld4(wf + (c + i) * 4);
    float a[4][4];
#pragma unroll
    for (int i = 0; i < 4; ++i) a[i][0] = a[i][1] = a[i][2] = a[i][3] = 0.f;
    const int64_t mbeg = (int64_t)blockIdx.x * rows_per_chunk, mend = min(M, mbeg + rows_per_chunk);
    constexpr int U = 4;
    if (act) {
        for (int64_t m0 = mbeg + slot; m0 < mend; m0 += (int64_t)U * RSL) {
            float4 vz[U], vx[U];
            bool ok[U];
#pragma unroll
            for (int u = 0; u < U; ++u) {
                const int64_t m = m0 + (int64_t)u * RSL;
                ok[u] = m < mend;
                const int64_t mc = ok[u] ? m : mbeg;
                vz[u] = ld4(dz + mc * C + c);
                vx[u] = xc[mc];
            }
#pragma unroll
            for (int u = 0; u < U; ++u) {
                if (!ok[u]) continue;
                const float g[4] = {vz[u].x, vz[u].y, vz[u].z, vz[u].w};
#pragma unroll
                for (int i = 0; i < 4; ++i) {
                    const float z = fmaf(k[i].z, vx[u].z, fmaf(k[i].y, vx[u].y, fmaf(k[i].x, vx[u].x, k[i].w)));
                    const float p = z > 0.f ? g[i] : 0.f;
                    a[i][0] = fmaf(p, vx[u].x, a[i][0]); a[i][1] = fmaf(p, vx[u].y, a[i][1]); a[i][2] = fmaf(p, vx[u].z, a[i][2]);
                    a[i][3] += p;
                }
            }
        }
    }
#pragma unroll
    for (int i = 0; i < 4; ++i)
#pragma unroll
        for (int j = 0; j < 4; ++j) red[tid * 16 + i * 4 + j] = act ? a[i][j] : 0.f;
    __syncthreads();
    float *out = partial + (int64_t)blockIdx.x * C * 4;
    for (int t = tid; t < C * 4; t += XYZ_T) {
// ... 61 lines not shown
        for (int k = 0; k < 3; ++k) {
            const double yx = w0 * Sxx[0][k] + w1 * Sxx[1][k] + w2 * Sxx[2][k] + (b - mu) * Sx[k];
            const float gk_ = (float)(sc * (T[k] - c1 * Sx[k] - c2 * is * yx));
            float *o = dw + (int64_t)c * ldw + xcol0 + k;
            *o = accumulate ? *o + gk_ : gk_;
        }
    }
}

}

using namespace papc;

extern "C" {

int papc_xyz_parts(int64_t M) { return M >= 1 ? (int)std::min<int64_t>(cdiv(M, 1024), XYZ_MAX_PARTS) : 0; }
int papc_xyz_bwd_parts(int64_t M) { return M >= 1 ? (int)cdiv(M, 1024) : 0; }

int papc_xyz_group_f32(const papc_group_src *grp, int B, float *xc, double *gram_partial, papc_stream_t stream)
{
    PAPC_REQUIRE(grp && grp->xyz && grp->new_xyz && xc && gram_partial, PAPC_E_INVALID, "papc_xyz_group_f32: null pointer");
    PAPC_REQUIRE(B >= 1 && grp->N >= 1 && grp->S >= 1 && grp->K >= 1, PAPC_E_INVALID, "papc_xyz_group_f32: bad sizes");
    PAPC_REQUIRE(aligned16(xc), PAPC_E_INVALID, "papc_xyz_group_f32: xc must be 16-byte aligned");
    const int64_t M = (int64_t)B * grp->S * grp->K;
    PAPC_REQUIRE(M < (1ll << 31), PAPC_E_UNSUPPORTED, "papc_xyz_group_f32: M=%lld >= 2^31 rows", (long long)M);
    GroupSrc g;
    memset(&g, 0, sizeof(g));
    g.xyz = grp->xyz; g.sb = grp->sb; g.sn = grp->sn; g.sc = grp->sc; g.new_xyz = grp->new_xyz; g.idx = grp->idx;
    g.N = grp->N; g.S = grp->S; g.K = grp->K; g.D = 0; g.xyz_first = 1;
    g.divK = make_fastdiv((uint32_t)grp->K); g.divS = make_fastdiv((uint32_t)grp->S);
    hipStream_t st = as_stream(stream);
    ProfScope prof(PAPC_K_GROUP, st);
    hipLaunchKernelGGL(xyz_group_kernel, dim3((unsigned)papc_xyz_parts(M)), dim3(XYZ_T), 0, st, g, M, reinterpret_cast<float4 *>(xc), gram_partial);
    return check_launch("papc_xyz_group_f32");
}

int papc_xyz_gram_fold_f32(const double *gram_partial, int parts, double *gram, papc_stream_t stream)
{
    PAPC_REQUIRE(gram_partial && gram && parts >= 1, PAPC_E_INVALID, "papc_xyz_gram_fold_f32: bad arguments");
    hipStream_t st = as_stream(stream);
    ProfScope prof(PAPC_K_GROUP, st);
    hipLaunchKernelGGL(xyz_gram_fold_kernel, dim3(1), dim3(256), 0, st, gram_partial, parts, gram);
    return check_launch("papc_xyz_gram_fold_f32");
}

int papc_xyz_l1_finalize_f32(const double *gram_partial, int parts, int64_t M, const float *w, int ldw, int xcol0, const float *bias,
                             const float *gamma, const float *beta, float eps, float momentum, int C, float *mean, float *invstd, float *scale,
                             float *shift, float *running_mean, float *running_var, float *wf, double *gram, papc_stream_t stream)
{
    PAPC_REQUIRE(gram_partial && w && mean && invstd && scale && shift && wf && gram, PAPC_E_INVALID, "papc_xyz_l1_finalize_f32: null pointer");
    PAPC_REQUIRE(parts >= 1 && M >= 1 && C >= 1 && ldw >= xcol0 + 3 && xcol0 >= 0, PAPC_E_INVALID, "papc_xyz_l1_finalize_f32: bad sizes");
    hipStream_t st = as_stream(stream);
    ProfScope prof(PAPC_K_MISC, st);
    hipLaunchKernelGGL(xyz_l1_finalize_kernel, dim3(1), dim3(256), 0, st, gram_partial, parts, (double)M, w, ldw, xcol0, bias, gamma, beta, eps,
                       momentum, C, mean, invstd, scale, shift, running_mean, running_var, wf, gram);
    return check_launch("papc_xyz_l1_finalize_f32");
}

int papc_xyz_l1_bwd_f32(const float *dz, const float *xc, const float *wf, int64_t M, int C, float *partial, papc_stream_t stream)
{
    PAPC_REQUIRE(dz && xc && wf && partial, PAPC_E_INVALID, "papc_xyz_l1_bwd_f32: null pointer");
    PAPC_REQUIRE(M >= 1 && C >= 4 && C <= 256 && C % 4 == 0, PAPC_E_UNSUPPORTED, "papc_xyz_l1_bwd_f32: C=%d must be a multiple of 4 in [4, 256]", C);
    PAPC_REQUIRE(aligned16(dz) && aligned16(xc) && aligned16(wf), PAPC_E_INVALID, "papc_xyz_l1_bwd_f32: 16-byte alignment");
    hipStream_t st = as_stream(stream);
    ProfScope prof(PAPC_K_BWD_DW, st);
    hipLaunchKernelGGL(xyz_l1_bwd_kernel, dim3((unsigned)papc_xyz_bwd_parts(M)), dim3(XYZ_T), 0, st, dz, reinterpret_cast<const float4 *>(xc), wf, M, C,
                       (int64_t)1024, partial);
    return check_launch("papc_xyz_l1_bwd_f32");
}

int papc_xyz_l1_bwd_finalize_f32(const float *partial, int parts, int64_t M, int C, const double *gram, const float *w, int ldw, int xcol0,
                                 const float *bias, const float *mean, const float *invstd, const float *scale, float *dgamma, float *dbeta,
                                 float *dw, int accumulate, papc_stream_t stream)
{
    PAPC_REQUIRE(partial && gram && w && mean && invstd && scale && dgamma && dbeta && dw, PAPC_E_INVALID, "papc_xyz_l1_bwd_finalize_f32: null pointer");
    PAPC_REQUIRE(parts >= 1 && M >= 1 && C >= 1 && C <= 256 && ldw >= xcol0 + 3 && xcol0 >= 0, PAPC_E_INVALID, "papc_xyz_l1_bwd_finalize_f32: bad sizes");
    hipStream_t st = as_stream(stream);
    ProfScope prof(PAPC_K_BWD_DW, st);
    hipLaunchKernelGGL(xyz_l1_bwd_finalize_kernel, dim3((unsigned)cdiv(C, 4)), dim3(1024), 0, st, partial, parts, (double)M, C, gram, w, ldw, xcol0, bias, mean, invstd,
                       scale, dgamma, dbeta, dw, accumulate);
    return check_launch("papc_xyz_l1_bwd_finalize_f32");
}

}
```

### papc_amd/mlp.py

```python
import ctypes

import torch

from . import _lib
from ._lib import BwdDy, BwdRed, GroupMax, GroupSrc, ReduceJob, ScatterDst, check, ptr, stream_ptr

A_PLAIN, A_BNRELU, A_GROUP, A_XYZ = 0, 1, 2, 6
DZ_DENSE, DZ_MAX = 0, 1


class StackSpec:

    def __init__(self, B, N, S, K, D, xyz_first, eps=1e-5, momentum=0.9, cut_gather_grad=False, pool=True, eval_bn=False):
        self.B, self.N, self.S, self.K, self.D = B, N, S, K, D
        self.pool = bool(pool)
        self.eval_bn = bool(eval_bn)
        self.xyz_first = bool(xyz_first)
        self.eps, self.momentum = float(eps), float(momentum)
        self.cut_gather_grad = cut_gather_grad
        self.M = B * S * K
        self.grad_targets = None
        self.wt_table = None
        self.xyz_pre = None
        self.compact = None
        self.plists = None


def _group_src(spec, xyz, new_xyz, feats, idx):
    g = GroupSrc()
    g.xyz = xyz.data_ptr()
    g.sb, g.sn, g.sc = xyz.stride(0), xyz.stride(1), xyz.stride(2)
    g.new_xyz = new_xyz.data_ptr()
    g.feats = ptr(feats)
    g.idx = ptr(idx)
    g.N, g.S, g.K, g.D = spec.N, spec.S, spec.K, spec.D
    g.xyz_first = int(spec.xyz_first)
    return g


import os
_FUSE_RED = os.environ.get("PAPC_NO_RED") != "1"
_FUSE_GMAX = os.environ.get("PAPC_NO_GMAX") != "1"
_RESIDENT_WGS = int(os.environ.get("PAPC_PARTS", "512"))
_LIN_GATHER = os.environ.get("PAPC_LIN_GATHER", "1") == "1"
_NOSTORE = os.environ.get("PAPC_NOSTORE", "1") == "1"
_SPARSE_MAX = os.environ.get("PAPC_SPARSE_MAX", "0") == "1"
_DW_WGS = int(os.environ.get("PAPC_DW_WGS", "512"))
_PY_ORCH = os.environ.get("PAPC_PY_ORCH", "0") == "1"
_XYZ1 = os.environ.get("PAPC_XYZ1", "1") == "1"
_XYZ_FUSE = os.environ.get("PAPC_XYZ_FUSE", "1") == "1"


def _dw_rows_per_chunk(M, cout, cin, min_rows=256):
    wide = 128 < cin <= 160
    tiles = ((cout + 127) // 128) * (1 if wide else (cin + 127) // 128)
    want = max(1, _DW_WGS // tiles)
    rpc = (M + want - 1) // want
    rpc = max(min_rows, ((rpc + 63) // 64) * 64)
    return rpc




def precompute_wt(weights, feat_blocks=()):
    lib = _lib.load()
    st = stream_ptr()
    table = {}
    ok = lambda w: w.is_cuda and w.is_contiguous() and w.dtype == torch.float32
    jobs = []
    for w in weights:
        if ok(w):
            cout = w.shape[0]
            cin = w.numel() // cout
            t = torch.empty(cin, cout, device=w.device, dtype=torch.float32)
            table[w.data_ptr()] = t
            jobs.append((w.data_ptr(), cin, t, cout, cin, 0))
    for w, xyz_first in feat_blocks:
        cout = w.shape[0]
        cin = w.numel() // cout
        if ok(w) and cin > 3:
            t = torch.empty(cout, cin - 3, device=w.device, dtype=torch.float32)
            table[("f", w.data_ptr())] = (t, bool(xyz_first))
            jobs.append((w.data_ptr() + (12 if xyz_first else 0), cin, t, cout, cin - 3, 1))
    for g0 in range(0, len(jobs), 8):
        grp = jobs[g0:g0 + 8]
        n = len(grp)
        srcs, dsts = (ctypes.c_void_p * n)(), (ctypes.c_void_p * n)()
        lds, rws, cls, cps = (ctypes.c_int * n)(), (ctypes.c_int * n)(), (ctypes.c_int * n)(), (ctypes.c_int * n)()
        for i, (src, ld, t, rows, cols, cp) in enumerate(grp):
            srcs[i], lds[i], dsts[i], rws[i], cls[i], cps[i] = src, ld, t.data_ptr(), rows, cols, cp
        check(lib.papc_transpose_batch_ld_f32(srcs, lds, dsts, rws, cls, cps, n, st), "papc_transpose_batch_ld_f32")
    return table


def xyz_first_layer_ok(M, c1, c2, n_layers):
    return bool(_XYZ1 and n_layers >= 3 and _lib.load().papc_mlp_xyz_ok(M, c1, c2))


def xyz_pregroup(xyz, new_xyz, idx, out=None):
    lib = _lib.load()
    B, N = xyz.shape[0], xyz.shape[1]
    S, K = idx.shape[1], idx.shape[2]
    M = B * S * K
    dev = xyz.device
    if out is None:
        out = (torch.empty(M, 4, device=dev, dtype=torch.float32), torch.empty(1, 16, device=dev, dtype=torch.float64))
    gpart = torch.empty(lib.papc_xyz_parts(M), 16, device=dev, dtype=torch.float64)
    g = GroupSrc()
    g.xyz = xyz.data_ptr()
    g.sb, g.sn, g.sc = xyz.stride(0), xyz.stride(1), xyz.stride(2)
    g.new_xyz, g.feats, g.idx = new_xyz.data_ptr(), 0, idx.data_ptr()
    g.N, g.S, g.K, g.D, g.xyz_first = N, S, K, 0, 1
    check(lib.papc_xyz_group_f32(ctypes.byref(g), B, ptr(out[0]), ptr(gpart), stream_ptr()), "papc_xyz_group_f32")
    check(lib.papc_xyz_gram_fold_f32(ptr(gpart), gpart.shape[0], ptr(out[1]), stream_ptr()), "papc_xyz_gram_fold_f32")
    return out


class SharedMLPMax(torch.autograd.Function):

    @staticmethod
    def forward(ctx, spec, bn_buffers, xyz, new_xyz, feats, idx, x_rows, *params):
        lib = _lib.load()
        st = stream_ptr()
        dev = params[0].device
        L = len(params) // 4
        M = spec.M
        parts = lib.papc_mlp_gemm_parts(M)
        plain = x_rows is not None
        grp = None if plain else _group_src(spec, xyz, new_xyz, feats, idx)
        ys, consts = [], []
        prev_y, prev_sc, prev_sh = None, None, None
        cin = x_rows.shape[1] if plain else spec.D + 3
        cin0 = cin
        ev = spec.eval_bn
        assert not ev or bn_buffers is not None, "eval_bn needs the running statistics"
        lin0 = (_LIN_GATHER and not ev and not plain and idx is not None and feats is not None and L >= 2 and spec.D % 4 == 0 and spec.D >= 16
                and params[0].shape[0] % 4 == 0 and params[0].shape[0] <= 256 and feats.is_contiguous())
        xyz1 = (not ev and not plain and idx is not None and feats is None and spec.D == 0
                and xyz_first_layer_ok(M, params[0].shape[0], params[4].shape[0] if L >= 2 else 0, L))
        xc = wf = gram = None
        cp = spec.compact if (lin0 and spec.pool and spec.compact is not None) else None
        if cp is not None:
            from . import compact as _cpm
            if not _cpm.stack_ok(M, spec.K, [params[4 * l].shape[0] for l in range(L)]):
                cp = None
        R_c = lib.papc_compact_corr_parts() if cp is not None else 0
        if cp is not None:
            grp.cidx, grp.seg_grp, grp.rows_dev = cp.cidx.data_ptr(), cp.seg_grp.data_ptr(), cp.rows.data_ptr()
        for l in range(L):
            w, b, gamma, beta = params[4 * l: 4 * l + 4]
            cout = w.shape[0]
            w2 = w.reshape(cout, cin)
            assert w2.is_contiguous()
            stats = None if ev else torch.empty(parts + R_c, 2, cout, device=dev, dtype=torch.float32)
            parts_l = parts
            gm_ref = None
            if cp is None and l == L - 1 and spec.pool and _FUSE_GMAX and not ev and lib.papc_mlp_gemm_gmax_ok(M, cout, spec.K):
                G_ = M // spec.K
                gbuf_f = torch.empty(2, G_, cout, device=dev, dtype=torch.float32)
                gbuf_i = torch.empty(2, G_, cout, device=dev, dtype=torch.int32)
                gm = GroupMax()
                gm.gmax, gm.gmin = gbuf_f[0].data_ptr(), gbuf_f[1].data_ptr()
                gm.amax, gm.amin = gbuf_i[0].data_ptr(), gbuf_i[1].data_ptr()
                gm.K = spec.K
                gm_ref = ctypes.byref(gm)
            if (gm_ref is not None and _NOSTORE and L >= 2 and l == L - 1 and prev_y is not None and not (l == 1 and xyz1)
                    and lib.papc_mlp_max_nostore_ok(M, cin, cout, spec.K)):
                y = None
            else:
                y = None if (l == 0 and xyz1) else torch.empty(M, cout, device=dev, dtype=torch.float32)
            if l == 0 and xyz1:
                y = stats = None
                nparts = 1
                if spec.xyz_pre is not None:
                    xc, gpart = spec.xyz_pre
                    assert tuple(xc.shape) == (M, 4) and tuple(gpart.shape) == (1, 16)
                else:
                    xc, gpart = xyz_pregroup(xyz, new_xyz, idx)
                cst = torch.empty(4, cout, device=dev, dtype=torch.float32)
                wf = torch.empty(cout, 4, device=dev, dtype=torch.float32)
                gram = torch.empty(16, device=dev, dtype=torch.float64)
                rm, rv = (bn_buffers[l] if bn_buffers is not None else (None, None))
                check(lib.papc_xyz_l1_finalize_f32(ptr(gpart), nparts, M, ptr(w2), cin, 0, ptr(b), ptr(gamma), ptr(beta), spec.eps, spec.momentum,
                                                   cout, cst[0].data_ptr(), cst[1].data_ptr(), cst[2].data_ptr(), cst[3].data_ptr(), ptr(rm), ptr(rv),
                                                   ptr(wf), ptr(gram), st), "papc_xyz_l1_finalize_f32")
                ys.append(None)
                consts.append(cst)
                prev_y, prev_sc, prev_sh = None, cst[2], cst[3]
                cin = cout
                continue
            if l == 1 and xyz1:
                check(lib.papc_mlp_gemm_f32(A_XYZ, ptr(xc), 4, None, ptr(wf), None, ptr(w2), ptr(b), M, cin, cout,
                                            ptr(y), ptr(stats), gm_ref, st), "papc_mlp_gemm_f32")
            elif l == 0 and plain:
                check(lib.papc_mlp_gemm_f32(A_PLAIN, ptr(x_rows), cin, None, None, None, ptr(w2), ptr(b), M, cin, cout,
                                            ptr(y), ptr(stats), gm_ref, st), "papc_mlp_gemm_f32")
            elif l == 0 and lin0:
                fcol0 = 3 if spec.xyz_first else 0
                wf = torch.empty(cout, spec.D, device=dev, dtype=torch.float32)
                check(lib.papc_copy2d_f32(w2.data_ptr() + 4 * fcol0, cin, ptr(wf), spec.D, cout, spec.D, 0, st), "papc_copy2d_f32")
                BN_ = spec.B * spec.N
                P = torch.empty(BN_, cout, device=dev, dtype=torch.float32)
                check(lib.papc_mlp_gemm_f32(A_PLAIN, ptr(feats), spec.D, None, None, None, ptr(wf), None, BN_, spec.D, cout, ptr(P), None,
                                            None, st), "papc_mlp_gemm_f32")
                parts_l = lib.papc_lingather_parts(M)
                stats = torch.empty(parts_l + R_c, 2, cout, device=dev, dtype=torch.float32)
                check(lib.papc_lingather_fwd_f32(ptr(P), ctypes.byref(grp), spec.B, ptr(w2), cin, 0 if spec.xyz_first else spec.D,
                                                 ptr(b), cout, ptr(y), ptr(stats), st), "papc_lingather_fwd_f32")
            elif l == 0:
                check(lib.papc_mlp_gemm_f32(A_GROUP, None, 0, ctypes.byref(grp), None, None, ptr(w2), ptr(b), M, cin, cout,
                                            ptr(y), ptr(stats), gm_ref, st), "papc_mlp_gemm_f32")
            elif cp is not None:
                check(lib.papc_mlp_gemm_rows_f32(A_BNRELU, ptr(prev_y), cin, None, ptr(prev_sc), ptr(prev_sh), ptr(w2), ptr(b), M, cin,
                                                 cout, ptr(y), ptr(stats), None, cp.rows.data_ptr(), st), "papc_mlp_gemm_rows_f32")
            else:
                check(lib.papc_mlp_gemm_f32(A_BNRELU, ptr(prev_y), cin, None, ptr(prev_sc), ptr(prev_sh), ptr(w2), ptr(b), M, cin,
                                            cout, ptr(y), ptr(stats), gm_ref, st), "papc_mlp_gemm_f32")
            if cp is not None:
                check(lib.papc_bn_stats_corr_f32(ptr(y), cout, cp.start.data_ptr(), cp.coef.data_ptr(), cp.G,
                                                 stats.data_ptr() + 4 * parts_l * 2 * cout, st), "papc_bn_stats_corr_f32")
                parts_l += R_c
            cst = torch.empty(4, cout, device=dev, dtype=torch.float32)
            rm, rv = (bn_buffers[l] if bn_buffers is not None else (None, None))
            if ev:
                check(lib.papc_bn_eval_consts_f32(ptr(rm), ptr(rv), ptr(gamma), ptr(beta), spec.eps, cout, cst[0].data_ptr(),
                                                  cst[1].data_ptr(), cst[2].data_ptr(), cst[3].data_ptr(), st), "papc_bn_eval_consts_f32")
            else:
                check(lib.papc_bn_finalize_f32(ptr(stats), parts_l, M, cout, ptr(gamma), ptr(beta), spec.eps, spec.momentum,
                                               cst[0].data_ptr(), cst[1].data_ptr(), cst[2].data_ptr(), cst[3].data_ptr(),
                                               ptr(rm), ptr(rv), st), "papc_bn_finalize_f32")
            ys.append(y)
            consts.append(cst)
            prev_y, prev_sc, prev_sh = y, cst[2], cst[3]
            cin = cout
        G = spec.B * spec.S
        argmax = None
        if not spec.pool:
            out = torch.empty(M, cin, device=dev, dtype=torch.float32)
# ... 336 lines not shown
```

### papc_amd/models.py

```python
import torch
import torch.nn as nn
import torch.nn.functional as F

from .layers import (PointNetFeaturePropagation, PointNetSetAbstraction, PointNetSetAbstractionMsg, _bn_buffers,
                     _stack_params)
from . import _lib
from . import head as _head
from .copyops import cat_copy
from .mlp import StackSpec, shared_mlp_max
from .plan import new_xyz

import os
_FUSED_HEAD = os.environ.get("PAPC_NO_FUSED_HEAD") != "1"


def _starts(start_idx, n):
    if start_idx is None:
        return [None] * n
    assert len(start_idx) == n, "start_idx must hold one [B] tensor per FPS level"
    return list(start_idx)


def _bn1d(bn, y):
    if not (bn.training and bn.track_running_stats and y.shape[0] > 1):
# ... 27 lines not shown
        logits = self.fc3(x)
        if labels is not None:
            return (_head.softmax_cross_entropy(logits, labels) if logits.is_cuda else F.cross_entropy(logits, labels.reshape(-1))), logits.detach()
        return logits


class PointNet2_SSG_Clas(nn.Module, _ClasHead):
    def __init__(self, name_scope='PointNet2_SSG_Clas_', num_classes=16, normal_channel=False, reference_quirks=False):
        super().__init__()
        in_channel = 6 if normal_channel else 3
        self.normal_channel = normal_channel
        q = dict(reference_quirks=reference_quirks)
        self.sa1 = PointNetSetAbstraction(npoint=512, radius=0.2, nsample=32, in_channel=in_channel, mlp=[64, 64, 128],
                                          group_all=False, **q)
        self.sa2 = PointNetSetAbstraction(npoint=128, radius=0.4, nsample=64, in_channel=128 + 3, mlp=[128, 128, 256],
                                          group_all=False, **q)
        self.sa3 = PointNetSetAbstraction(npoint=None, radius=None, nsample=None, in_channel=256 + 3,
                                          mlp=[256, 512, 1024], group_all=True, **q)
        self.fc1 = nn.Linear(1024, 512)
        self.bn1 = nn.BatchNorm1d(512)
        self.drop1 = nn.Dropout(0.4)
        self.fc2 = nn.Linear(512, 256)
        self.bn2 = nn.BatchNorm1d(256)
        self.drop2 = nn.Dropout(0.4)
        self.fc3 = nn.Linear(256, num_classes)

    def plan_sampling(self, inputs, start_idx=None, out=None, stage=None):
        xyz = torch.as_tensor(inputs)
        if self.normal_channel:
            xyz = xyz[:, :3, :]
        s = _starts(start_idx, 2)
        with torch.no_grad():
            o = out if out is not None else (None, None)
            if stage == "fps1":
                return self.sa1.sample_fps(xyz, s[0], out=new_xyz(o[0]))
            p1 = self.sa1.sample(xyz, s[0], out=o[0], new_xyz=new_xyz(o[0]) if stage == "rest" else None)
            p2 = self.sa2.sample(new_xyz(p1).transpose(1, 2), s[1], out=o[1])
        return p1, p2

    def forward(self, inputs, start_idx=None, plan=None, after_sa2=None, tap=None, after_sa3=None, labels=None, after_sa1=None):
        xyz = torch.as_tensor(inputs)
        B = xyz.shape[0]
        if self.normal_channel:
            norm, xyz = xyz[:, 3:, :], xyz[:, :3, :]
        else:
            norm = None
        s = _starts(start_idx, 2)
        pl = plan if plan is not None else (None, None)
        wt = None
        if torch.is_grad_enabled() and xyz.is_cuda:
            from . import smallm
            from .mlp import precompute_wt
            ws = [c.weight for c in list(self.sa1.mlp_convs)[1:]] + [c.weight for c in self.sa2.mlp_convs]
            if not (smallm.takes_group_all(B, self.sa2.npoint, [c.weight.shape[0] for c in self.sa3.mlp_convs])):
                ws += [c.weight for c in self.sa3.mlp_convs]
            wt = precompute_wt(ws, feat_blocks=[(self.sa2.mlp_convs[0].weight, True)])
        l1_xyz, l1_points = self.sa1(xyz, norm, s[0], sampled=pl[0], wt_table=wt)
        if after_sa1 is not None:
            after_sa1()
        l2_xyz, l2_points = self.sa2(l1_xyz, l1_points, s[1], sampled=pl[1], wt_table=wt)
        if after_sa2 is not None:
            after_sa2()
        if tap is not None:
            tap["l2_points"] = l2_points
        l3_xyz, l3_points = self.sa3(l2_xyz, l2_points, wt_table=wt)
        if after_sa3 is not None:
            after_sa3()
        x = l3_points.reshape(B, 1024)
        return self._head(x, labels)


class PointNet2_MSG_Clas(nn.Module, _ClasHead):
    def __init__(self, name_scope='PointNet2_MSG_Clas_', num_classes=16, normal_channel=False, reference_quirks=False):
        super().__init__()
        in_channel = 3 if normal_channel else 0
        self.normal_channel = normal_channel
        q = dict(reference_quirks=reference_quirks)
        self.sa1 = PointNetSetAbstractionMsg(512, [0.1, 0.2, 0.4], [16, 32, 128], in_channel,
                                             [[32, 32, 64], [64, 64, 128], [64, 96, 128]], **q)
        self.sa2 = PointNetSetAbstractionMsg(128, [0.2, 0.4, 0.8], [32, 64, 128], 320,
                                             [[64, 64, 128], [128, 128, 256], [128, 128, 256]], **q)
        self.sa3 = PointNetSetAbstraction(None, None, None, 640 + 3, [256, 512, 1024], True, **q)
        self.fc1 = nn.Linear(1024, 512)
        self.bn1 = nn.BatchNorm1d(512)
        self.drop1 = nn.Dropout(0.4)
        self.fc2 = nn.Linear(512, 256)
        self.bn2 = nn.BatchNorm1d(256)
        self.drop2 = nn.Dropout(0.5)
        self.fc3 = nn.Linear(256, num_classes)

    def forward(self, inputs, start_idx=None):
        xyz = torch.as_tensor(inputs)
        B = xyz.shape[0]
        if self.normal_channel:
            norm, xyz = xyz[:, 3:, :], xyz[:, :3, :]
        else:
            norm = None
        s = _starts(start_idx, 2)
        l1_xyz, l1_points = self.sa1(xyz, norm, s[0])
        l2_xyz, l2_points = self.sa2(l1_xyz, l1_points, s[1])
        l3_xyz, l3_points = self.sa3(l2_xyz, l2_points)
        x = l3_points.reshape(B, 1024)
        return self._head(x)


class PointNet_Basic_Clas(nn.Module):

    reference_names = {"convs.0": "mlp_1.0", "bns.0": "mlp_1.1", "convs.1": "mlp_1.3", "bns.1": "mlp_1.4", "convs.2": "mlp_2.0",
                       "bns.2": "mlp_2.1", "convs.3": "mlp_2.3", "bns.3": "mlp_2.4", "convs.4": "mlp_2.6", "bns.4": "mlp_2.7"}
# ... 297 lines not shown
```

### papc_amd/smallm.py

```python
import ctypes
import os

import torch

from . import _lib
from ._lib import check, ptr, stream_ptr

PLAIN, CONCAT, BNRELU, DY_DENSE, DY_MAX = 0, 1, 2, 3, 4
DZ_DENSE = 0
EPI_STORE, EPI_FWD, EPI_FWD_GMAX, EPI_RED = 0, 1, 2, 3
K_MLP_GEMM, K_BWD_DX, K_BWD_DW = 3, 6, 7
GROUP = 128
ENABLED = os.environ.get("PAPC_PLANES", "1") == "1"
MAX_ROWS = int(os.environ.get("PAPC_PLANES_MAXROWS", "16384"))
POINTWISE = os.environ.get("PAPC_PLANES_POINTWISE", "1") == "1"

c_p, c_i, c_l, c_f = ctypes.c_void_p, ctypes.c_int, ctypes.c_int64, ctypes.c_float


class PgWJob(ctypes.Structure):
    _fields_ = [("src", c_p), ("row_stride", c_l), ("col_stride", c_l), ("R", c_i), ("K", c_i), ("planes", c_p)]


class PgPrep(ctypes.Structure):
# ... 23 lines not shown
        return False
    if spec.pool and spec.K != GROUP:
        return False
    if not spec.pool and (x_rows is None or not POINTWISE):
        return False
    if len(params) < 8:
        return False
    couts = [params[4 * l].shape[0] for l in range(len(params) // 4)]
    if any(c % 8 for c in couts):
        return False
    if x_rows is not None:
        return x_rows.is_cuda and x_rows.is_contiguous() and x_rows.shape[1] % 8 == 0 and x_rows.dtype == torch.float32
    if xyz is None or not xyz.is_cuda or spec.S != 1:
        return False
    return feats is None or (feats.is_contiguous() and feats.dtype == torch.float32)


def takes_group_all(B, n_points, couts):
    M = B * n_points
    return bool(ENABLED and n_points == GROUP and M <= MAX_ROWS and len(couts) >= 2 and not any(c % 8 for c in couts))


def _planes(lib, R, K, dev):
    return torch.empty(lib.papc_pg_planes_bytes(R, K), dtype=torch.uint8, device=dev)


def _split_for(R1, R2, nst):
    tiles = ((R1 + 127) // 128) * ((R2 + 127) // 128)
    s = 1
    min_stages = 2 if tiles <= 2 else 8
    while s * 2 * tiles <= 256 and nst % (s * 2) == 0 and nst // (s * 2) >= min_stages:
        s *= 2
    return s


class PlanesMLPMax(torch.autograd.Function):

    @staticmethod
    def forward(ctx, spec, bn_buffers, xyz, new_xyz, feats, idx, x_rows, *params):
        lib = _lib.load()
        st = stream_ptr()
        dev = params[0].device
        L = len(params) // 4
        M = spec.M
        T = M // GROUP
        plain = x_rows is not None
        cin0 = x_rows.shape[1] if plain else spec.D + 3
        ch = [cin0] + [params[4 * l].shape[0] for l in range(L)]
        want_bwd = any(ctx.needs_input_grad)
        in_grad = (plain and x_rows.requires_grad) or ((not plain) and feats is not None and feats.requires_grad and not spec.cut_gather_grad)
        fcol0 = (3 if spec.xyz_first else 0) if not plain else 0
        n_in = cin0 if plain else spec.D

        w2s, wp, wtp, jobs = [], [], [None] * L, []
        for l in range(L):
            w2 = params[4 * l].reshape(ch[l + 1], ch[l])
            assert w2.is_contiguous()
            w2s.append(w2)
            wp.append(_planes(lib, ch[l + 1], ch[l], dev))
            jobs.append((w2.data_ptr(), ch[l], 1, ch[l + 1], ch[l], wp[l].data_ptr()))
            if want_bwd and (l > 0 or in_grad):
                rows, off = (ch[l], 0) if l > 0 else (n_in, fcol0)
                wtp[l] = _planes(lib, rows, ch[l + 1], dev)
                jobs.append((w2.data_ptr() + 4 * off, 1, ch[l], rows, ch[l + 1], wtp[l].data_ptr()))
        for j0 in range(0, len(jobs), 8):
            chunk = jobs[j0:j0 + 8]
            arr = (PgWJob * len(chunk))()
            for a, (src, sr, sc, R, K, dst) in zip(arr, chunk):
                a.src, a.row_stride, a.col_stride, a.R, a.K, a.planes = src, sr, sc, R, K, dst
            check(lib.papc_pg_prep_weights_f32(arr, len(chunk), st), "papc_pg_prep_weights_f32")

        def prep(**kw):
            a = PgPrep()
            for k, v in kw.items():
                setattr(a, k, v)
            check(lib.papc_pg_prep_rows_f32(ctypes.byref(a), st), "papc_pg_prep_rows_f32")

        P = _planes(lib, M, cin0, dev)
        PT = [None] * L
        if want_bwd:
            PT[0] = _planes(lib, cin0, M, dev)
        if plain:
            prep(mode=PLAIN, M=M, C=cin0, x=x_rows.data_ptr(), ldx=cin0, planes=P.data_ptr(), planes_t=ptr(PT[0]))
        else:
            prep(mode=CONCAT, M=M, C=cin0, xyz=xyz.data_ptr(), sb=xyz.stride(0), sn=xyz.stride(1), sc=xyz.stride(2), feats=ptr(feats),
                 N=spec.N, D=spec.D, xyz_first=int(spec.xyz_first), planes=P.data_ptr(), planes_t=ptr(PT[0]))
        ys, consts = [], []
        gbuf_f = gbuf_i = None
        for l in range(L):
            cout = ch[l + 1]
            y = torch.empty(M, cout, device=dev, dtype=torch.float32)
            stats = torch.empty(T, 2, cout, device=dev, dtype=torch.float32)
            cst = torch.empty(4, cout, device=dev, dtype=torch.float32)
            g = PgGemm()
            g.epi = EPI_FWD_GMAX if (l == L - 1 and spec.pool) else EPI_FWD
            g.a, g.b, g.R1, g.R2, g.K = P.data_ptr(), wp[l].data_ptr(), M, cout, ch[l]
            g.c, g.ldc, g.split, g.split_stride = y.data_ptr(), cout, 1, 0
            g.bias, g.stats, g.family = ptr(params[4 * l + 1]), stats.data_ptr(), K_MLP_GEMM
            if l == L - 1 and spec.pool:
                gbuf_f = torch.empty(2, T, cout, device=dev, dtype=torch.float32)
                gbuf_i = torch.empty(2, T, cout, device=dev, dtype=torch.int32)
                g.gmax, g.gmin, g.amax, g.amin = gbuf_f[0].data_ptr(), gbuf_f[1].data_ptr(), gbuf_i[0].data_ptr(), gbuf_i[1].data_ptr()
            check(lib.papc_pg_gemm_f32(ctypes.byref(g), st), "papc_pg_gemm_f32")
            rm, rv = (bn_buffers[l] if bn_buffers is not None else (None, None))
            gamma, beta = params[4 * l + 2], params[4 * l + 3]
            if l < L - 1:
                P = _planes(lib, M, cout, dev)
                if want_bwd:
                    PT[l + 1] = _planes(lib, cout, M, dev)
                prep(mode=BNRELU, M=M, C=cout, x=y.data_ptr(), ldx=cout, stats=stats.data_ptr(), parts=T, gamma=ptr(gamma), beta=ptr(beta),
                     eps=spec.eps, momentum=spec.momentum, running_mean=ptr(rm), running_var=ptr(rv), mean=cst[0].data_ptr(),
# ... 132 lines not shown
```

### papc_amd/stack.py

```python
import ctypes
import os

import torch

from . import _lib
from ._lib import check, ptr, stream_ptr

MAXL = 8
c_p, c_i, c_l, c_f = ctypes.c_void_p, ctypes.c_int32, ctypes.c_int64, ctypes.c_float
NO_LINGATHER, NO_XYZ1, NO_NOSTORE, NO_GMAX, NO_FUSED_RED, NO_COMPACT, NO_PLANES, NO_PLANES_POINTWISE, NO_XYZ_FUSE, NO_WSTATS, NO_PSEL, NO_GSIGN = 1, 2, 4, 8, 16, 32, 64, 128, 256, 512, 1024, 2048


class SaDesc(ctypes.Structure):
    _fields_ = [("B", c_i), ("N", c_i), ("S", c_i), ("K", c_i), ("D", c_i), ("n_layers", c_i), ("cin", c_i), ("cout", c_i * MAXL),
                ("input", c_i), ("identity_rows", c_i), ("xyz_first", c_i), ("pool", c_i), ("eval_bn", c_i), ("cut_gather_grad", c_i),
                ("eps", c_f), ("momentum", c_f), ("disable", ctypes.c_uint32), ("inference", c_i), ("want_input_grad", c_i)]


class SaLayer(ctypes.Structure):
    _fields_ = [("w", c_p), ("b", c_p), ("gamma", c_p), ("beta", c_p), ("running_mean", c_p), ("running_var", c_p)]


class CompactSrc(ctypes.Structure):
    _fields_ = [("start", c_p), ("rows", c_p), ("cidx", c_p), ("seg_grp", c_p), ("wrow", c_p), ("coef", c_p), ("G", c_i)]


class SaIo(ctypes.Structure):
    _fields_ = [("xyz", c_p), ("sb", c_l), ("sn", c_l), ("sc", c_l), ("new_xyz", c_p), ("feats", c_p), ("idx", c_p), ("x_rows", c_p),
                ("xc", c_p), ("xc_gram", c_p), ("compact", ctypes.POINTER(CompactSrc)), ("consts3", c_p), ("consts3_ld", c_i),
                ("layer", SaLayer * MAXL), ("out", c_p), ("saved", c_p), ("scratch", c_p), ("plists", c_p), ("wfeat", c_p)]


class SaPlan(ctypes.Structure):
    _fields_ = [("d", SaDesc), ("cin0", c_i), ("lin0", c_i), ("xyz1", c_i), ("gmax", c_i), ("nostore", c_i), ("compact", c_i), ("sparse_max", c_i),
                ("planes", c_i), ("saved_bytes", c_l), ("fwd_scratch_bytes", c_l), ("bwd_scratch_bytes", c_l), ("off_y", c_l * MAXL), ("off_cst", c_l * MAXL),
                ("off_argmax", c_l)]


class SaGrads(ctypes.Structure):
    _fields_ = [("gout", c_p), ("dw", c_p * MAXL), ("db", c_p * MAXL), ("dgamma", c_p * MAXL), ("dbeta", c_p * MAXL), ("acc_w", c_i * MAXL),
                ("acc_gb", c_i * MAXL), ("wt", c_p * MAXL), ("grad_feats", c_p), ("grad_x", c_p), ("defer", c_p)]


_CONSTS3 = {}
LAST_PLANS = {}


def _consts3(dev):
    t = _CONSTS3.get(str(dev))
    if t is None:
        mk = lambda: torch.tensor([1.0, 0.0, 1e30], device=dev, dtype=torch.float32).view(3, 1).expand(3, 1024).contiguous()
        if _lib._capturing():
            return mk()
        t = _CONSTS3[str(dev)] = mk()
    return t


def _disable_bits():
    from . import mlp
    bits = 0
    if not mlp._LIN_GATHER: bits |= NO_LINGATHER
    if not mlp._XYZ1: bits |= NO_XYZ1
    if not mlp._NOSTORE: bits |= NO_NOSTORE
    if not mlp._FUSE_GMAX: bits |= NO_GMAX
    if not mlp._FUSE_RED: bits |= NO_FUSED_RED
    from . import smallm
    if not smallm.ENABLED: bits |= NO_PLANES
    if not smallm.POINTWISE: bits |= NO_PLANES_POINTWISE
    if not mlp._XYZ_FUSE: bits |= NO_XYZ_FUSE
    if os.environ.get("PAPC_GSIGN", "1") == "0": bits |= NO_GSIGN
    if os.environ.get("PAPC_PSEL", "1") == "0": bits |= NO_PSEL
    if os.environ.get("PAPC_WSTATS", "1") == "0": bits |= NO_WSTATS
    return bits


def _fill_io(io, spec, xyz, new_xyz, feats, idx, x_rows, params, bn_buffers, keep):
    L = len(params) // 4
    if x_rows is None:
        io.xyz = xyz.data_ptr()
        io.sb, io.sn, io.sc = xyz.stride(0), xyz.stride(1), xyz.stride(2)
        io.new_xyz, io.feats, io.idx = new_xyz.data_ptr(), ptr(feats), ptr(idx)
    else:
        io.x_rows = x_rows.data_ptr()
    if spec.xyz_pre is not None:
        io.xc, io.xc_gram = spec.xyz_pre[0].data_ptr(), spec.xyz_pre[1].data_ptr()
    cp = spec.compact
    if cp is not None:
        src = CompactSrc(cp.start.data_ptr(), cp.rows.data_ptr(), cp.cidx.data_ptr(), cp.seg_grp.data_ptr(), cp.wrow.data_ptr(), cp.coef.data_ptr(), cp.G)
        keep.append(src)
        io.compact = ctypes.pointer(src)
    pl = getattr(spec, "plists", None)
    if pl is not None:
        src = _lib.PointLists(pl.prange.data_ptr(), pl.prow.data_ptr(), pl.pmeta.data_ptr(), int(pl.compact),
                              pl.pmom.data_ptr() if getattr(pl, "pmom", None) is not None else None)
        keep.append(src)
        keep.append(pl)
        io.plists = ctypes.addressof(src)
    wtab = getattr(spec, "wt_table", None)
    if wtab is not None and feats is not None and L >= 1:
        ent = wtab.get(("f", params[0].data_ptr()))
        cin0 = params[0].numel() // params[0].shape[0]
        if ent is not None and ent[1] == bool(spec.xyz_first) and tuple(ent[0].shape) == (params[0].shape[0], cin0 - 3) and cin0 - 3 == spec.D:
            io.wfeat = ent[0].data_ptr()
            keep.append(ent[0])
    c3 = _consts3(params[0].device)
    keep.append(c3)
    io.consts3, io.consts3_ld = c3.data_ptr(), c3.shape[1]
    for l in range(L):
        w, b, gamma, beta = params[4 * l: 4 * l + 4]
        ly = io.layer[l]
        assert w.is_contiguous()
        ly.w, ly.b, ly.gamma, ly.beta = w.data_ptr(), ptr(b), gamma.data_ptr(), beta.data_ptr()
        if bn_buffers is not None:
            ly.running_mean, ly.running_var = ptr(bn_buffers[l][0]), ptr(bn_buffers[l][1])


class SharedMLPStack(torch.autograd.Function):

    @staticmethod
    def forward(ctx, spec, bn_buffers, xyz, new_xyz, feats, idx, x_rows, *params):
        lib = _lib.load()
        dev = params[0].device
        L = len(params) // 4
        assert 1 <= L <= MAXL
        plain = x_rows is not None
        d = SaDesc()
        d.B, d.N, d.S, d.K, d.D, d.n_layers = spec.B, spec.N, spec.S, spec.K, spec.D, L
        d.cin = x_rows.shape[1] if plain else spec.D + 3
        for l in range(L):
            d.cout[l] = params[4 * l].shape[0]
        d.input = 1 if plain else 0
        d.identity_rows = int((not plain) and idx is None)
        d.xyz_first, d.pool, d.eval_bn, d.cut_gather_grad = int(spec.xyz_first), int(spec.pool), int(spec.eval_bn), int(bool(spec.cut_gather_grad))
        d.eps, d.momentum = spec.eps, spec.momentum
        d.disable = _disable_bits()
        if feats is not None and not feats.is_contiguous():
            d.disable |= NO_LINGATHER | NO_PLANES
        if plain and not x_rows.is_contiguous():
            d.disable |= NO_PLANES
        d.inference = int(not any(ctx.needs_input_grad))
        d.want_input_grad = int((plain and x_rows.requires_grad) or ((not plain) and feats is not None and feats.requires_grad and not spec.cut_gather_grad))
        keep = []
        io = SaIo()
        _fill_io(io, spec, xyz, new_xyz, feats, idx, x_rows, params, bn_buffers, keep)
        plan = SaPlan()
        check(lib.papc_sa_mlp_plan(ctypes.byref(d), ctypes.byref(io), ctypes.byref(plan)), "papc_sa_mlp_plan")
        M = spec.M
        G = spec.B * spec.S
        cL = params[4 * (L - 1)].shape[0]
        out = torch.empty(G if spec.pool else M, cL, device=dev, dtype=torch.float32)
        saved = torch.empty(plan.saved_bytes, device=dev, dtype=torch.uint8)
        scratch = torch.empty(plan.fwd_scratch_bytes, device=dev, dtype=torch.uint8)
        io.out, io.saved, io.scratch = out.data_ptr(), saved.data_ptr(), scratch.data_ptr()
        check(lib.papc_sa_mlp_fwd(ctypes.byref(plan), ctypes.byref(io), stream_ptr()), "papc_sa_mlp_fwd")
        ctx.spec, ctx.L, ctx.plan, ctx.saved = spec, L, plan, saved
        LAST_PLANS[(int(M), tuple(int(d.cout[l]) for l in range(L)))] = dict(
            lin0=bool(plan.lin0), xyz1=bool(plan.xyz1), gmax=bool(plan.gmax), nostore=bool(plan.nostore), compact=bool(plan.compact), planes=bool(plan.planes),
            xyz_fuse=bool(plan.xyz1) and not (d.disable & NO_XYZ_FUSE))
        ctx.compact = spec.compact if plan.compact else None
        ctx.nostore, ctx.xyz1, ctx.lin0, ctx.planes = bool(plan.nostore), bool(plan.xyz1), bool(plan.lin0), bool(plan.planes)
        ctx.bn_buffers = bn_buffers
        ctx.wt_table = spec.wt_table
        ctx.feats_needs_grad = feats is not None and feats.requires_grad and not spec.cut_gather_grad
        ctx.x_needs_grad = plain and x_rows.requires_grad
        ctx.save_for_backward(xyz, new_xyz, feats, idx, x_rows, *params)
        return out

    @staticmethod
    def views(ctx):
        plan, saved, spec, L = ctx.plan, ctx.saved, ctx.spec, ctx.L
        M, G = spec.M, spec.B * spec.S
        def view(off, n, dt):
            return None if off < 0 else saved[off: off + 4 * n].view(dt)
        cs = [plan.d.cout[l] for l in range(L)]
        am = view(plan.off_argmax, G * cs[-1], torch.int32)
        ys = [None if plan.off_y[l] < 0 else view(plan.off_y[l], M * cs[l], torch.float32).view(M, cs[l]) for l in range(L)]
        cst = [view(plan.off_cst[l], 4 * cs[l], torch.float32).view(4, cs[l]) for l in range(L)]
        return (None if am is None else am.view(G, cs[-1])), ys, cst

    @staticmethod
    def backward(ctx, gout):
        lib = _lib.load()
        spec, L, plan = ctx.spec, ctx.L, ctx.plan
        tens = ctx.saved_tensors
        xyz, new_xyz, feats, idx, x_rows = tens[:5]
        params = tens[5:]
        dev = gout.device
        gout = gout.contiguous().float()
        keep = []
        io = SaIo()
        _fill_io(io, spec, xyz, new_xyz, feats, idx, x_rows, params, ctx.bn_buffers, keep)
        scratch = torch.empty(plan.bwd_scratch_bytes, device=dev, dtype=torch.uint8)
        io.saved, io.scratch = ctx.saved.data_ptr(), scratch.data_ptr()
        g = SaGrads()
        g.gout = gout.data_ptr()
        grads = [None] * (4 * L)
        all_inplace = True
        for l in range(L):
            w = params[4 * l]
            cout = w.shape[0]
            cin = w.numel() // cout
            tgt = spec.grad_targets[4 * l: 4 * l + 4] if spec.grad_targets is not None else None
            inplace = tgt is not None and all(t is not None for t in tgt)
            gb_inplace = tgt is not None and tgt[2] is not None and tgt[3] is not None and not spec.eval_bn
            all_inplace = all_inplace and inplace
            if inplace:
                g.dw[l], g.db[l], g.acc_w[l] = tgt[0].data_ptr(), tgt[1].data_ptr(), 1
            else:
                dw = torch.empty(cout, cin, device=dev, dtype=torch.float32)
                grads[4 * l] = dw.reshape(w.shape)
                g.dw[l], g.acc_w[l] = dw.data_ptr(), 0
                if tgt is not None and tgt[1] is not None and not spec.eval_bn:
                    g.db[l] = None
                else:
                    db = torch.empty(cout, device=dev, dtype=torch.float32)
                    grads[4 * l + 1] = db
                    g.db[l] = db.data_ptr()
            if gb_inplace and not (l == 0 and plan.xyz1 and not inplace):
                g.dgamma[l], g.dbeta[l], g.acc_gb[l] = tgt[2].data_ptr(), tgt[3].data_ptr(), 1
            else:
                dgb = torch.empty(2, cout, device=dev, dtype=torch.float32)
                grads[4 * l + 2], grads[4 * l + 3] = dgb[0], dgb[1]
                g.dgamma[l], g.dbeta[l], g.acc_gb[l] = dgb[0].data_ptr(), dgb[1].data_ptr(), 0
            if ctx.wt_table is not None:
                t = ctx.wt_table.get(w.data_ptr())
                if t is not None and tuple(t.shape) == (cin, cout):
                    g.wt[l] = t.data_ptr()
        grad_feats = grad_x = None
        if ctx.feats_needs_grad:
            grad_feats = torch.empty(spec.B, spec.N, spec.D, device=dev, dtype=torch.float32)
# ... 11 lines not shown
```

Measured before the change: 21530.

## Merge weight transposes, plane prep and first-layer BN finalize into one prologue launch

Adds a single prologue kernel that runs, in one launch, the weight transposes, the bf16x3 plane packing of weights, and the closed-form BN finalize of the xyz-first layer. These were previously separate launches issued inside the SA stacks. The results are handed to later stages through the weight table so they can skip their own prep. The aim is fewer small kernel launches and less per-call host work. It adds handover plumbing and shape checks, and a knob falls back to separate launches.

```diff
diff --git a/include/papc_hip.h b/include/papc_hip.h
--- a/include/papc_hip.h
+++ b/include/papc_hip.h
@@ -250,6 +250,8 @@
     void *saved, *scratch;
     const papc_point_lists *plists;
     const float *wfeat;
+    float *l1_cst, *l1_wf; double *l1_gram;
+    const void *wplanes[PAPC_SA_MAX_LAYERS], *wtplanes[PAPC_SA_MAX_LAYERS];
 } papc_sa_io;
 typedef struct papc_sa_plan {
     papc_sa_desc d;
@@ -512,6 +514,16 @@
 int papc_transpose_batch_ld_f32(const float *const *src, const int *src_ld, float *const *dst, const int *rows, const int *cols, const int *copy, int count,
                                 papc_stream_t stream);
 
+typedef struct papc_xyz_l1_fin {
+    const double *gram_partial; int32_t parts; int64_t M;
+    const float *w; int32_t ldw, xcol0;
+    const float *bias, *gamma, *beta; float eps, momentum; int32_t C;
+    float *mean, *invstd, *scale, *shift, *running_mean, *running_var, *wf;
+    double *gram;
+} papc_xyz_l1_fin;
+int papc_weight_prologue_f32(const float *const *src, const int *src_ld, float *const *dst, const int *rows, const int *cols, const int *copy,
+                             int n_transpose, const papc_pg_wjob *planes, int n_planes, const papc_xyz_l1_fin *fin, papc_stream_t stream);
+
 int papc_fill_f32(float *p, int64_t n, float value, papc_stream_t stream);
 int papc_copy2d_f32(const float *src, int64_t src_ld, float *dst, int64_t dst_ld, int rows, int cols, int transpose,
                     papc_stream_t stream);
diff --git a/papc_amd/_lib.py b/papc_amd/_lib.py
--- a/papc_amd/_lib.py
+++ b/papc_amd/_lib.py
@@ -169,6 +169,7 @@
     "papc_pg_fold_f32": (c_i, [c_p, c_i, c_p]),
     "papc_transpose_batch_f32": (c_i, [c_p, c_p, c_p, c_p, c_i, c_p]),
     "papc_transpose_batch_ld_f32": (c_i, [c_p, c_p, c_p, c_p, c_p, c_p, c_i, c_p]),
+    "papc_weight_prologue_f32": (c_i, [c_p, c_p, c_p, c_p, c_p, c_p, c_i, c_p, c_i, c_p, c_p]),
     "papc_rotate_nms_f32": (c_i, [c_p, c_i, c_f, c_p, c_p, c_p, ctypes.c_size_t, c_p]),
     "papc_rotate_iou_f32": (c_i, [c_p, c_p, c_i, c_i, c_i, c_p, c_p]),
     "papc_rbbox_iou_f32": (c_i, [c_p, c_p, c_p, c_f, c_i, c_i, c_p, c_p]),
@@ -217,6 +218,12 @@
     return _lib
 
 
+def knob(name):
+    v = c_i()
+    check(load().papc_knob_get(name.encode(), ctypes.byref(v)), "papc_knob_get")
+    return v.value
+
+
 def check(status, what):
     if status != 0:
         msg = load().papc_last_error_string().decode("utf-8", "replace")
diff --git a/papc_amd/build.py b/papc_amd/build.py
--- a/papc_amd/build.py
+++ b/papc_amd/build.py
@@ -15,7 +15,7 @@
           "-I", os.path.join(ROOT, "include"), "-I", CSRC, "-Wall", "-Wno-unused-function"]
 NOSLP = ["-fno-slp-vectorize"]
 RES = ["-Rpass-analysis=kernel-resource-usage"]
-EXTRA = {"mlp_stream.hip": NOSLP + RES, "mlp_gemm.hip": NOSLP, "mlp_dw.hip": NOSLP, "sampling.hip": NOSLP, "bn_ops.hip": NOSLP, "folds.hip": NOSLP, "pfn.hip": NOSLP, "interp.hip": NOSLP, "nms.hip": NOSLP, "head.hip": NOSLP, "lingather.hip": NOSLP, "smallm.hip": NOSLP + RES}
+EXTRA = {"mlp_stream.hip": NOSLP + RES, "mlp_gemm.hip": NOSLP, "mlp_dw.hip": NOSLP, "sampling.hip": NOSLP, "bn_ops.hip": NOSLP, "folds.hip": NOSLP, "pfn.hip": NOSLP, "interp.hip": NOSLP, "nms.hip": NOSLP, "head.hip": NOSLP, "lingather.hip": NOSLP, "smallm.hip": NOSLP + RES, "prologue.hip": NOSLP}
 
 
 def _hipcc():
diff --git a/papc_amd/csrc/bn_ops.hip b/papc_amd/csrc/bn_ops.hip
--- a/papc_amd/csrc/bn_ops.hip
+++ b/papc_amd/csrc/bn_ops.hip
@@ -1,4 +1,5 @@
 #include "common.h"
+#include "prologue.h"
 
 namespace papc {
 
@@ -507,40 +508,9 @@
     }
 }
 
-struct TransposeBatch {
-    const float *src[8];
-    float *dst[8];
-    int rows[8], cols[8];
-    int ld[8], copy[8];
-};
-
 __global__ __launch_bounds__(256) void transpose_batch_kernel(TransposeBatch t)
 {
-    __shared__ float tile[32][33];
-    const int m = blockIdx.y;
-    const int rows = t.rows[m], cols = t.cols[m];
-    const int tiles_c = (cols + 31) >> 5, tiles = ((rows + 31) >> 5) * tiles_c;
-    const float *__restrict__ src = t.src[m];
-    float *__restrict__ dst = t.dst[m];
-    const int tx = threadIdx.x & 31, ty = threadIdx.x >> 5;
-    for (int tl = blockIdx.x; tl < tiles; tl += gridDim.x) {
-        const int r0 = (tl / tiles_c) * 32, c0 = (tl % tiles_c) * 32;
-#pragma unroll
-        for (int i = 0; i < 4; ++i) {
-            const int r = r0 + ty + 8 * i, c = c0 + tx;
-            const float v = (r < rows && c < cols) ? src[(int64_t)r * t.ld[m] + c] : 0.f;
-            tile[ty + 8 * i][tx] = v;
-            if (t.copy[m] && r < rows && c < cols) dst[(int64_t)r * cols + c] = v;
-        }
-        if (t.copy[m]) continue;
-        __syncthreads();
-#pragma unroll
-        for (int i = 0; i < 4; ++i) {
-            const int c = c0 + ty + 8 * i, r = r0 + tx;
-            if (r < rows && c < cols) dst[(int64_t)c * rows + r] = tile[tx][ty + 8 * i];
-        }
-        __syncthreads();
-    }
+    transpose_batch_body(t, (int)blockIdx.y, (int)blockIdx.x, (int)gridDim.x);
 }
 
 }
diff --git a/papc_amd/csrc/capi.hip b/papc_amd/csrc/capi.hip
--- a/papc_amd/csrc/capi.hip
+++ b/papc_amd/csrc/capi.hip
@@ -69,6 +69,7 @@
     {"PAPC_LGL_VARIANT", 0, 0, 3},
     {"PAPC_LG_PP", 1, 0, 1},
     {"PAPC_PG_GROUP", 1, 0, 1},
+    {"PAPC_LAUNCH_MERGE", 1, 0, 15},
 };
 static int g_knobs[KNOB_COUNT];
 static int knob_parse(int id, const char *e)
@@ -174,6 +175,7 @@
     PAPC_SIZEOF(papc_pg_gemm)
     PAPC_SIZEOF(papc_pg_fold_job)
     PAPC_SIZEOF(papc_copy_job)
+    PAPC_SIZEOF(papc_xyz_l1_fin)
 #undef PAPC_SIZEOF
     return -1;
 }
diff --git a/papc_amd/csrc/common.h b/papc_amd/csrc/common.h
--- a/papc_amd/csrc/common.h
+++ b/papc_amd/csrc/common.h
@@ -24,9 +24,10 @@
 enum Knob {
     KNOB_LG_PARTS, KNOB_DW_F32, KNOB_DW_DBG, KNOB_DW_XYZ, KNOB_PARTS, KNOB_GEMM_F32, KNOB_GEMM_WAVES, KNOB_MAXCAT_WAVES,
     KNOB_GEMM_WS, KNOB_GEMM_OCC, KNOB_GEMM_DBG, KNOB_GEMM_KB, KNOB_GEMM_MINWG, KNOB_GEMM_TL, KNOB_FPS_THREADS,
-    KNOB_FPS_THREADS_SMALL, KNOB_STREAM, KNOB_STREAM_MINTILES, KNOB_STREAM_CK, KNOB_STREAM_ASM, KNOB_PFN_MFMA, KNOB_DW_RS64, KNOB_DW_ROWS, KNOB_DW_ROWS_BLOCKS, KNOB_DW_ROWSX, KNOB_PG_DBG, KNOB_PG_NB, KNOB_PG_NS, KNOB_STREAM_MAXCAT, KNOB_MAX_NOSTORE, KNOB_PFN_FUSED_TAILS, KNOB_STREAM_NW12, KNOB_LG_LISTS, KNOB_FOLD_WAVES, KNOB_LGL_VARIANT, KNOB_LG_PP, KNOB_PG_GROUP, KNOB_COUNT
+    KNOB_FPS_THREADS_SMALL, KNOB_STREAM, KNOB_STREAM_MINTILES, KNOB_STREAM_CK, KNOB_STREAM_ASM, KNOB_PFN_MFMA, KNOB_DW_RS64, KNOB_DW_ROWS, KNOB_DW_ROWS_BLOCKS, KNOB_DW_ROWSX, KNOB_PG_DBG, KNOB_PG_NB, KNOB_PG_NS, KNOB_STREAM_MAXCAT, KNOB_MAX_NOSTORE, KNOB_PFN_FUSED_TAILS, KNOB_STREAM_NW12, KNOB_LG_LISTS, KNOB_FOLD_WAVES, KNOB_LGL_VARIANT, KNOB_LG_PP, KNOB_PG_GROUP, KNOB_LAUNCH_MERGE, KNOB_COUNT
 };
 int knob(int id);
+enum { MERGE_WEIGHT_PROLOGUE = 1 };
 
 struct ProfScope {
     int kernel;
diff --git a/papc_amd/csrc/prologue.h b/papc_amd/csrc/prologue.h
--- /dev/null
+++ b/papc_amd/csrc/prologue.h
@@ -0,0 +1,122 @@
+#pragma once
+#include "bf16x3.h"
+
+namespace papc {
+
+__host__ __device__ static inline int64_t ru64(int64_t a, int64_t b) { return (a + b - 1) / b * b; }
+
+struct TransposeBatch {
+    const float *src[8];
+    float *dst[8];
+    int rows[8], cols[8];
+    int ld[8], copy[8];
+};
+
+__device__ __forceinline__ void transpose_batch_body(const TransposeBatch &t, int m, int bx, int nbx)
+{
+    __shared__ float tile[32][33];
+    const int rows = t.rows[m], cols = t.cols[m];
+    const int tiles_c = (cols + 31) >> 5, tiles = ((rows + 31) >> 5) * tiles_c;
+    const float *__restrict__ src = t.src[m];
+    float *__restrict__ dst = t.dst[m];
+    const int tx = threadIdx.x & 31, ty = threadIdx.x >> 5;
+    for (int tl = bx; tl < tiles; tl += nbx) {
+        const int r0 = (tl / tiles_c) * 32, c0 = (tl % tiles_c) * 32;
+#pragma unroll
+        for (int i = 0; i < 4; ++i) {
+            const int r = r0 + ty + 8 * i, c = c0 + tx;
+            const float v = (r < rows && c < cols) ? src[(int64_t)r * t.ld[m] + c] : 0.f;
+            tile[ty + 8 * i][tx] = v;
+            if (t.copy[m] && r < rows && c < cols) dst[(int64_t)r * cols + c] = v;
+        }
+        if (t.copy[m]) continue;
+        __syncthreads();
+#pragma unroll
+        for (int i = 0; i < 4; ++i) {
+            const int c = c0 + ty + 8 * i, r = r0 + tx;
+            if (r < rows && c < cols) dst[(int64_t)c * rows + r] = tile[tx][ty + 8 * i];
+        }
+        __syncthreads();
+    }
+}
+
+__device__ __forceinline__ void store_planes8(char *frag0, int slot, const float (&v)[8])
+{
+    bf16x8 pl[3];
+    split8(v, pl);
+    *reinterpret_cast<uint4 *>(frag0 + slot * 16) = __builtin_bit_cast(uint4, pl[0]);
+    *reinterpret_cast<uint4 *>(frag0 + 1024 + slot * 16) = __builtin_bit_cast(uint4, pl[1]);
+    *reinterpret_cast<uint4 *>(frag0 + 2048 + slot * 16) = __builtin_bit_cast(uint4, pl[2]);
+}
+
+struct WJob {
+    const float *src; int64_t sr, sc;
+    int R, K;
+    char *dst;
+};
+struct WJobs {
+    WJob j[8];
+};
+
+__device__ __forceinline__ void pg_prep_w_body(const WJob &jb, int bx, int nbx)
+{
+    const int KB = (int)(ru64(jb.K, 32) / 16), RB = (int)(ru64(jb.R, 32) / 32);
+    const int lane = threadIdx.x & 63, wv = threadIdx.x >> 6;
+    const int r_in = lane & 31, h = lane >> 5;
+    for (int f = bx * 4 + wv; f < RB * KB; f += nbx * 4) {
+        const int rb = f / KB, kb = f - rb * KB;
+        const int r = rb * 32 + r_in, k0 = kb * 16 + h * 8;
+        float v[8];
+#pragma unroll
+        for (int i = 0; i < 8; ++i) v[i] = (r < jb.R && k0 + i < jb.K) ? jb.src[(int64_t)r * jb.sr + (int64_t)(k0 + i) * jb.sc] : 0.f;
+        store_planes8(jb.dst + ((int64_t)rb * KB + kb) * 3072, lane, v);
+    }
+}
+
+struct XyzL1Fin {
+    const double *partial; int parts; double M;
+    const float *w; int ldw, xcol0;
+    const float *bias, *gamma, *beta; float eps, momentum; int C;
+    float *mean, *invstd, *scale, *shift, *rmean, *rvar, *wf;
+    double *gram;
+};
+
+__device__ __forceinline__ void xyz_l1_finalize_body(const XyzL1Fin &a)
+{
+    __shared__ double red[16][16];
+    __shared__ double G[10];
+    const int e = threadIdx.x & 15, sl = threadIdx.x >> 4;
+    double s = 0.0;
+    if (e < 10) for (int t = sl; t < a.parts; t += 16) s += a.partial[(int64_t)t * 16 + e];
+    red[sl][e] = s;
+    __syncthreads();
+    if (threadIdx.x < 10) {
+        double v = 0.0;
+#pragma unroll
+        for (int q = 0; q < 16; ++q) v += red[q][threadIdx.x];
+        G[threadIdx.x] = v;
+        a.gram[threadIdx.x] = v;
+    }
+    __syncthreads();
+    const double M = a.M;
+    for (int c = threadIdx.x; c < a.C; c += 256) {
+        const double w0 = a.w[(int64_t)c * a.ldw + a.xcol0], w1 = a.w[(int64_t)c * a.ldw + a.xcol0 + 1], w2 = a.w[(int64_t)c * a.ldw + a.xcol0 + 2];
+        const double b = a.bias ? (double)a.bias[c] : 0.0;
+        const double mx = G[0] / M, my = G[1] / M, mz = G[2] / M;
+        const double cxx = G[3] / M - mx * mx, cxy = G[4] / M - mx * my, cxz = G[5] / M - mx * mz;
+        const double cyy = G[6] / M - my * my, cyz = G[7] / M - my * mz, czz = G[8] / M - mz * mz;
+        const double mu = w0 * mx + w1 * my + w2 * mz + b;
+        double var = w0 * (w0 * cxx + w1 * cxy + w2 * cxz) + w1 * (w0 * cxy + w1 * cyy + w2 * cyz) + w2 * (w0 * cxz + w1 * cyz + w2 * czz);
+        if (var < 0.0) var = 0.0;
+        const double is = 1.0 / sqrt(var + (double)a.eps);
+        const double sc = (a.gamma ? (double)a.gamma[c] : 1.0) * is;
+        const double sh = (a.beta ? (double)a.beta[c] : 0.0) - mu * sc;
+        a.mean[c] = (float)mu; a.invstd[c] = (float)is; a.scale[c] = (float)sc; a.shift[c] = (float)sh;
+        if (a.rmean) a.rmean[c] = a.momentum * a.rmean[c] + (1.f - a.momentum) * (float)mu;
+        if (a.rvar) a.rvar[c] = a.momentum * a.rvar[c] + (1.f - a.momentum) * (float)var;
+        a.wf[c * 4 + 0] = (float)(sc * w0); a.wf[c * 4 + 1] = (float)(sc * w1); a.wf[c * 4 + 2] = (float)(sc * w2);
+        a.wf[c * 4 + 3] = (float)(sc * b + sh);
+    }
+}
+
+}
diff --git a/papc_amd/csrc/prologue.hip b/papc_amd/csrc/prologue.hip
--- /dev/null
+++ b/papc_amd/csrc/prologue.hip
@@ -0,0 +1,81 @@
+#include "prologue.h"
+
+namespace papc {
+
+struct WeightPrologue {
+    TransposeBatch t; int nt;
+    WJobs w; int nw;
+    XyzL1Fin f;
+};
+
+__global__ __launch_bounds__(256) void weight_prologue_kernel(WeightPrologue p)
+{
+    const int y = (int)blockIdx.y, bx = (int)blockIdx.x, nbx = (int)gridDim.x;
+    if (y < p.nt) transpose_batch_body(p.t, y, bx, nbx);
+    else if (y < p.nt + p.nw) pg_prep_w_body(p.w.j[y - p.nt], bx, nbx);
+    else if (bx == 0) xyz_l1_finalize_body(p.f);
+}
+
+}
+
+using namespace papc;
+
+extern "C" {
+
+int papc_weight_prologue_f32(const float *const *src, const int *src_ld, float *const *dst, const int *rows, const int *cols, const int *copy,
+                             int n_transpose, const papc_pg_wjob *planes, int n_planes, const papc_xyz_l1_fin *fin, papc_stream_t stream)
+{
+    PAPC_REQUIRE(n_transpose >= 0 && n_transpose <= 8 && n_planes >= 0 && n_planes <= 8, PAPC_E_INVALID,
+                 "papc_weight_prologue_f32: %d transposes, %d plane jobs (0..8 each)", n_transpose, n_planes);
+    PAPC_REQUIRE(n_transpose || n_planes || fin, PAPC_E_INVALID, "papc_weight_prologue_f32: nothing to do");
+    PAPC_REQUIRE(!n_transpose || (src && dst && rows && cols), PAPC_E_INVALID, "papc_weight_prologue_f32: null transpose table");
+    PAPC_REQUIRE(!n_planes || planes, PAPC_E_INVALID, "papc_weight_prologue_f32: null plane jobs");
+    if (!(knob(KNOB_LAUNCH_MERGE) & MERGE_WEIGHT_PROLOGUE) || (n_transpose > 0) + (n_planes > 0) + (fin != nullptr) == 1) {
+        if (n_transpose) {
+            const int rc = papc_transpose_batch_ld_f32(src, src_ld, dst, rows, cols, copy, n_transpose, stream);
+            if (rc != PAPC_OK) return rc;
+        }
+        if (fin) {
+            const int rc = papc_xyz_l1_finalize_f32(fin->gram_partial, fin->parts, fin->M, fin->w, fin->ldw, fin->xcol0, fin->bias, fin->gamma, fin->beta, fin->eps,
+                                                    fin->momentum, fin->C, fin->mean, fin->invstd, fin->scale, fin->shift, fin->running_mean, fin->running_var,
+                                                    fin->wf, fin->gram, stream);
+            if (rc != PAPC_OK) return rc;
+        }
+        if (n_planes) return papc_pg_prep_weights_f32(planes, n_planes, stream);
+        return PAPC_OK;
+    }
+    WeightPrologue p;
+    memset(&p, 0, sizeof(p));
+    int64_t nbx = 1;
+    p.nt = n_transpose;
+    for (int i = 0; i < n_transpose; ++i) {
+        PAPC_REQUIRE(src[i] && dst[i] && rows[i] >= 1 && cols[i] >= 1, PAPC_E_INVALID, "papc_weight_prologue_f32: bad transpose entry %d", i);
+        p.t.src[i] = src[i]; p.t.dst[i] = dst[i]; p.t.rows[i] = rows[i]; p.t.cols[i] = cols[i];
+        p.t.ld[i] = src_ld ? src_ld[i] : cols[i]; p.t.copy[i] = copy ? copy[i] : 0;
+        PAPC_REQUIRE(p.t.ld[i] >= cols[i], PAPC_E_INVALID, "papc_weight_prologue_f32: transpose entry %d: row stride shorter than a row", i);
+        nbx = std::max<int64_t>(nbx, std::min<int64_t>(cdiv(rows[i], 32) * cdiv(cols[i], 32), 512));
+    }
+    p.nw = n_planes;
+    for (int i = 0; i < n_planes; ++i) {
+        PAPC_REQUIRE(planes[i].src && planes[i].planes && planes[i].R >= 1 && planes[i].K >= 1, PAPC_E_INVALID, "papc_weight_prologue_f32: bad plane job %d", i);
+        PAPC_REQUIRE(aligned16(planes[i].planes), PAPC_E_INVALID, "papc_weight_prologue_f32: planes must be 16-byte aligned");
+        WJob &j = p.w.j[i];
+        j.src = planes[i].src; j.sr = planes[i].row_stride; j.sc = planes[i].col_stride; j.R = planes[i].R; j.K = planes[i].K;
+        j.dst = reinterpret_cast<char *>(planes[i].planes);
+        nbx = std::max<int64_t>(nbx, std::min<int64_t>(cdiv((ru64(j.R, 32) / 32) * (ru64(j.K, 32) / 16), 4), 512));
+    }
+    if (fin) {
+        PAPC_REQUIRE(fin->gram_partial && fin->w && fin->mean && fin->invstd && fin->scale && fin->shift && fin->wf && fin->gram, PAPC_E_INVALID,
+                     "papc_weight_prologue_f32: null pointer in the first-layer finalize");
+        PAPC_REQUIRE(fin->parts >= 1 && fin->M >= 1 && fin->C >= 1 && fin->ldw >= fin->xcol0 + 3 && fin->xcol0 >= 0, PAPC_E_INVALID,
+                     "papc_weight_prologue_f32: bad sizes in the first-layer finalize");
+        p.f = XyzL1Fin{fin->gram_partial, fin->parts, (double)fin->M, fin->w, fin->ldw, fin->xcol0, fin->bias, fin->gamma, fin->beta, fin->eps, fin->momentum,
+                       fin->C, fin->mean, fin->invstd, fin->scale, fin->shift, fin->running_mean, fin->running_var, fin->wf, fin->gram};
+    }
+    hipStream_t st = as_stream(stream);
+    ProfScope prof(PAPC_K_MISC, st);
+    hipLaunchKernelGGL(weight_prologue_kernel, dim3((unsigned)nbx, (unsigned)(n_transpose + n_planes + (fin ? 1 : 0))), dim3(256), 0, st, p);
+    return check_launch("papc_weight_prologue_f32");
+}
+
+}
diff --git a/papc_amd/csrc/sa_mlp.hip b/papc_amd/csrc/sa_mlp.hip
--- a/papc_amd/csrc/sa_mlp.hip
+++ b/papc_amd/csrc/sa_mlp.hip
@@ -268,6 +268,18 @@
     return c.off;
 }
 
+static bool planes_handed_over(const papc_sa_plan &p, const papc_sa_io &io, PlanesSaved &s, PlanesFwd *f)
+{
+    const int L = p.d.n_layers;
+    for (int l = 0; l < L; ++l)
+        if (!io.wplanes[l] || (s.wtp[l] && !io.wtplanes[l])) return false;
+    for (int l = 0; l < L; ++l) {
+        if (f) f->wp[l] = const_cast<void *>(io.wplanes[l]);
+        if (s.wtp[l]) s.wtp[l] = const_cast<void *>(io.wtplanes[l]);
+    }
+    return true;
+}
+
 static int planes_fwd(const papc_sa_plan &p, const papc_sa_io &io, papc_stream_t st)
 {
     const papc_sa_desc &d = p.d;
@@ -277,7 +289,7 @@
     PlanesSaved s; PlanesFwd f;
     layout_planes_saved(p, io.saved, s);
     layout_planes_fwd(p, io.scratch, f);
-    {
+    if (!planes_handed_over(p, io, s, &f)) {
         papc_pg_wjob jobs[2 * PAPC_SA_MAX_LAYERS];
         int n = 0;
         const int fcol0 = plain ? 0 : (d.xyz_first ? 3 : 0);
@@ -343,6 +355,7 @@
     PlanesSaved s; PlanesBwd b;
     layout_planes_saved(p, io.saved, s);
     layout_planes_bwd(p, io.scratch, b);
+    planes_handed_over(p, io, s, nullptr);
     int cmaxc = 0;
     for (int l = 0; l < L; ++l) cmaxc = std::max(cmaxc, d.cout[l]);
     float *grad_in = plain ? gr.grad_x : gr.grad_feats;
@@ -506,6 +519,8 @@
     SavedPtrs s; FwdPtrs f;
     layout_saved(p, io->saved, s);
     layout_fwd(p, io->scratch, f);
+    const bool l1_done = p.xyz1 && io->l1_cst && io->l1_wf && io->l1_gram;
+    if (l1_done) { s.cst[0] = io->l1_cst; s.wf = io->l1_wf; s.gram = io->l1_gram; }
     const int parts = papc_mlp_gemm_parts(M);
     const bool wstats = p.compact && !(d.disable & PAPC_SA_NO_WSTATS);
     const int R_c = (p.compact && !wstats) ? papc_compact_corr_parts() : 0;
@@ -544,8 +559,9 @@
                 SA_CALL(papc_xyz_gram_fold_f32(f.gpart + 16, papc_xyz_parts(M), f.gpart, st));
                 xc = s.xc; gpart1 = f.gpart;
             }
-            SA_CALL(papc_xyz_l1_finalize_f32(gpart1, 1, M, ly.w, cin, 0, ly.b, ly.gamma, ly.beta, d.eps, d.momentum, cout, cst, cst + cout, cst + 2 * cout,
-                                             cst + 3 * cout, ly.running_mean, ly.running_var, s.wf, s.gram, st));
+            if (!l1_done)
+                SA_CALL(papc_xyz_l1_finalize_f32(gpart1, 1, M, ly.w, cin, 0, ly.b, ly.gamma, ly.beta, d.eps, d.momentum, cout, cst, cst + cout, cst + 2 * cout,
+                                                 cst + 3 * cout, ly.running_mean, ly.running_var, s.wf, s.gram, st));
             prev_y = nullptr; prev_sc = cst + 2 * cout; prev_sh = cst + 3 * cout;
             cin = cout;
             continue;
@@ -601,6 +617,7 @@
     SavedPtrs s; BwdPtrs b;
     layout_saved(p, io->saved, s);
     layout_bwd(p, io->scratch, b);
+    if (p.xyz1 && io->l1_cst && io->l1_wf && io->l1_gram) { s.cst[0] = io->l1_cst; s.wf = io->l1_wf; s.gram = io->l1_gram; }
     const float *xc = p.xyz1 ? ((io->xc && io->xc_gram) ? io->xc : s.xc) : nullptr;
     papc_group_src grp;
     if (!plain) fill_grp(grp, d, *io, p.compact);
diff --git a/papc_amd/csrc/smallm.hip b/papc_amd/csrc/smallm.hip
--- a/papc_amd/csrc/smallm.hip
+++ b/papc_amd/csrc/smallm.hip
@@ -1,45 +1,15 @@
 #include "fold.h"
 #include "mlp_loaders.h"
+#include "prologue.h"
 
 namespace papc {
 
 enum { PG_EPI_STORE = 0, PG_EPI_FWD = 1, PG_EPI_FWD_GMAX = 2, PG_EPI_RED = 3 };
 enum { PG_PREP_PLAIN = 0, PG_PREP_CONCAT = 1, PG_PREP_BNRELU = 2, PG_PREP_DY_DENSE = 3, PG_PREP_DY_MAX = 4 };
 
-__host__ __device__ static inline int64_t ru64(int64_t a, int64_t b) { return (a + b - 1) / b * b; }
-
-__device__ __forceinline__ void store_planes8(char *frag0, int slot, const float (&v)[8])
-{
-    bf16x8 pl[3];
-    split8(v, pl);
-    *reinterpret_cast<uint4 *>(frag0 + slot * 16) = __builtin_bit_cast(uint4, pl[0]);
-    *reinterpret_cast<uint4 *>(frag0 + 1024 + slot * 16) = __builtin_bit_cast(uint4, pl[1]);
-    *reinterpret_cast<uint4 *>(frag0 + 2048 + slot * 16) = __builtin_bit_cast(uint4, pl[2]);
-}
-
-struct WJob {
-    const float *src; int64_t sr, sc;
-    int R, K;
-    char *dst;
-};
-struct WJobs {
-    WJob j[8];
-};
-
 __global__ __launch_bounds__(256) void pg_prep_w_kernel(WJobs jobs)
 {
-    const WJob jb = jobs.j[blockIdx.y];
-    const int KB = (int)(ru64(jb.K, 32) / 16), RB = (int)(ru64(jb.R, 32) / 32);
-    const int lane = threadIdx.x & 63, wv = threadIdx.x >> 6;
-    const int r_in = lane & 31, h = lane >> 5;
-    for (int f = blockIdx.x * 4 + wv; f < RB * KB; f += gridDim.x * 4) {
-        const int rb = f / KB, kb = f - rb * KB;
-        const int r = rb * 32 + r_in, k0 = kb * 16 + h * 8;
-        float v[8];
-#pragma unroll
-        for (int i = 0; i < 8; ++i) v[i] = (r < jb.R && k0 + i < jb.K) ? jb.src[(int64_t)r * jb.sr + (int64_t)(k0 + i) * jb.sc] : 0.f;
-        store_planes8(jb.dst + ((int64_t)rb * KB + kb) * 3072, lane, v);
-    }
+    pg_prep_w_body(jobs.j[blockIdx.y], (int)blockIdx.x, (int)gridDim.x);
 }
 
 struct PrepArgs {
diff --git a/papc_amd/csrc/xyz1.hip b/papc_amd/csrc/xyz1.hip
--- a/papc_amd/csrc/xyz1.hip
+++ b/papc_amd/csrc/xyz1.hip
@@ -1,4 +1,5 @@
 #include "mlp_loaders.h"
+#include "prologue.h"
 
 namespace papc {
 
@@ -62,45 +63,9 @@
     }
 }
 
-__global__ __launch_bounds__(256) void xyz_l1_finalize_kernel(const double *__restrict__ partial, int parts, double M, const float *__restrict__ w, int ldw,
-                                                              int xcol0, const float *__restrict__ bias, const float *__restrict__ gamma,
-                                                              const float *__restrict__ beta, float eps, float momentum, int C, float *mean,
-                                                              float *invstd, float *scale, float *shift, float *rmean, float *rvar, float *wf,
-                                                              double *gram)
-{
-    __shared__ double red[16][16];
-    __shared__ double G[10];
-    const int e = threadIdx.x & 15, sl = threadIdx.x >> 4;
-    double s = 0.0;
-    if (e < 10) for (int t = sl; t < parts; t += 16) s += partial[(int64_t)t * 16 + e];
-    red[sl][e] = s;
-    __syncthreads();
-    if (threadIdx.x < 10) {
-        double v = 0.0;
-#pragma unroll
-        for (int q = 0; q < 16; ++q) v += red[q][threadIdx.x];
-        G[threadIdx.x] = v;
-        gram[threadIdx.x] = v;
-    }
-    __syncthreads();
-    for (int c = threadIdx.x; c < C; c += 256) {
-        const double w0 = w[(int64_t)c * ldw + xcol0], w1 = w[(int64_t)c * ldw + xcol0 + 1], w2 = w[(int64_t)c * ldw + xcol0 + 2];
-        const double b = bias ? (double)bias[c] : 0.0;
-        const double mx = G[0] / M, my = G[1] / M, mz = G[2] / M;
-        const double cxx = G[3] / M - mx * mx, cxy = G[4] / M - mx * my, cxz = G[5] / M - mx * mz;
-        const double cyy = G[6] / M - my * my, cyz = G[7] / M - my * mz, czz = G[8] / M - mz * mz;
-        const double mu = w0 * mx + w1 * my + w2 * mz + b;
-        double var = w0 * (w0 * cxx + w1 * cxy + w2 * cxz) + w1 * (w0 * cxy + w1 * cyy + w2 * cyz) + w2 * (w0 * cxz + w1 * cyz + w2 * czz);
-        if (var < 0.0) var = 0.0;
-        const double is = 1.0 / sqrt(var + (double)eps);
-        const double sc = (gamma ? (double)gamma[c] : 1.0) * is;
-        const double sh = (beta ? (double)beta[c] : 0.0) - mu * sc;
-        mean[c] = (float)mu; invstd[c] = (float)is; scale[c] = (float)sc; shift[c] = (float)sh;
-        if (rmean) rmean[c] = momentum * rmean[c] + (1.f - momentum) * (float)mu;
-        if (rvar) rvar[c] = momentum * rvar[c] + (1.f - momentum) * (float)var;
-        wf[c * 4 + 0] = (float)(sc * w0); wf[c * 4 + 1] = (float)(sc * w1); wf[c * 4 + 2] = (float)(sc * w2);
-        wf[c * 4 + 3] = (float)(sc * b + sh);
-    }
+__global__ __launch_bounds__(256) void xyz_l1_finalize_kernel(XyzL1Fin a)
+{
+    xyz_l1_finalize_body(a);
 }
 
 __global__ __launch_bounds__(XYZ_T) void xyz_l1_bwd_kernel(const float *__restrict__ dz, const float4 *__restrict__ xc, const float *__restrict__ wf,
@@ -268,8 +233,8 @@
     PAPC_REQUIRE(parts >= 1 && M >= 1 && C >= 1 && ldw >= xcol0 + 3 && xcol0 >= 0, PAPC_E_INVALID, "papc_xyz_l1_finalize_f32: bad sizes");
     hipStream_t st = as_stream(stream);
     ProfScope prof(PAPC_K_MISC, st);
-    hipLaunchKernelGGL(xyz_l1_finalize_kernel, dim3(1), dim3(256), 0, st, gram_partial, parts, (double)M, w, ldw, xcol0, bias, gamma, beta, eps,
-                       momentum, C, mean, invstd, scale, shift, running_mean, running_var, wf, gram);
+    XyzL1Fin a{gram_partial, parts, (double)M, w, ldw, xcol0, bias, gamma, beta, eps, momentum, C, mean, invstd, scale, shift, running_mean, running_var, wf, gram};
+    hipLaunchKernelGGL(xyz_l1_finalize_kernel, dim3(1), dim3(256), 0, st, a);
     return check_launch("papc_xyz_l1_finalize_f32");
 }
 
diff --git a/papc_amd/mlp.py b/papc_amd/mlp.py
--- a/papc_amd/mlp.py
+++ b/papc_amd/mlp.py
@@ -62,7 +62,7 @@
 
 
 
-def precompute_wt(weights, feat_blocks=()):
+def precompute_wt(weights, feat_blocks=(), planes=(), l1=None):
     lib = _lib.load()
     st = stream_ptr()
     table = {}
@@ -82,15 +82,73 @@
             t = torch.empty(cout, cin - 3, device=w.device, dtype=torch.float32)
             table[("f", w.data_ptr())] = (t, bool(xyz_first))
             jobs.append((w.data_ptr() + (12 if xyz_first else 0), cin, t, cout, cin - 3, 1))
-    for g0 in range(0, len(jobs), 8):
-        grp = jobs[g0:g0 + 8]
+    merge = bool(_lib.knob("PAPC_LAUNCH_MERGE") & 1)
+    pjobs = []
+    fin = None
+    if merge:
+        from .smallm import PgWJob, _planes
+        for w, wt in planes:
+            if not ok(w):
+                continue
+            cout = w.shape[0]
+            cin = w.numel() // cout
+            t = _planes(lib, cout, cin, w.device)
+            table[("p", w.data_ptr())] = (t, (cout, cin, 0))
+            pjobs.append((w.data_ptr(), cin, 1, cout, cin, t))
+            if wt is not None:
+                rows, off = (cin, 0) if wt is True else wt
+                t = _planes(lib, rows, cout, w.device)
+                table[("pt", w.data_ptr())] = (t, (rows, cout, off))
+                pjobs.append((w.data_ptr() + 4 * off, 1, cin, rows, cout, t))
+        if l1 is not None and ok(l1[0]):
+            w, b, gamma, beta, bufs, eps, momentum, M, gram_in = l1
+            C = w.shape[0]
+            cst = torch.empty(4, C, device=w.device, dtype=torch.float32)
+            wf = torch.empty(C, 4, device=w.device, dtype=torch.float32)
+            gram = torch.empty(16, device=w.device, dtype=torch.float64)
+            rm, rv = bufs if bufs is not None else (None, None)
+            fin = XyzL1Fin(gram_in.data_ptr(), 1, M, w.data_ptr(), w.numel() // C, 0, ptr(b), ptr(gamma), ptr(beta), eps, momentum, C, cst[0].data_ptr(),
+                           cst[1].data_ptr(), cst[2].data_ptr(), cst[3].data_ptr(), ptr(rm), ptr(rv), wf.data_ptr(), gram.data_ptr())
+            table[("l1", w.data_ptr())] = (cst, wf, gram)
+    first = True
+    for g0 in range(0, max(len(jobs), len(pjobs), 1), 8):
+        grp, pgrp = jobs[g0:g0 + 8], pjobs[g0:g0 + 8]
         n = len(grp)
-        srcs, dsts = (ctypes.c_void_p * n)(), (ctypes.c_void_p * n)()
-        lds, rws, cls, cps = (ctypes.c_int * n)(), (ctypes.c_int * n)(), (ctypes.c_int * n)(), (ctypes.c_int * n)()
+        srcs, dsts = (ctypes.c_void_p * max(n, 1))(), (ctypes.c_void_p * max(n, 1))()
+        lds, rws, cls, cps = (ctypes.c_int * max(n, 1))(), (ctypes.c_int * max(n, 1))(), (ctypes.c_int * max(n, 1))(), (ctypes.c_int * max(n, 1))()
         for i, (src, ld, t, rows, cols, cp) in enumerate(grp):
             srcs[i], lds[i], dsts[i], rws[i], cls[i], cps[i] = src, ld, t.data_ptr(), rows, cols, cp
-        check(lib.papc_transpose_batch_ld_f32(srcs, lds, dsts, rws, cls, cps, n, st), "papc_transpose_batch_ld_f32")
+        f = fin if first else None
+        first = False
+        if not pgrp and f is None:
+            if n:
+                check(lib.papc_transpose_batch_ld_f32(srcs, lds, dsts, rws, cls, cps, n, st), "papc_transpose_batch_ld_f32")
+            continue
+        arr = (PgWJob * max(len(pgrp), 1))()
+        for a, (src, sr, sc, R, K, t) in zip(arr, pgrp):
+            a.src, a.row_stride, a.col_stride, a.R, a.K, a.planes = src, sr, sc, R, K, t.data_ptr()
+        check(lib.papc_weight_prologue_f32(srcs, lds, dsts, rws, cls, cps, n, arr, len(pgrp), ctypes.byref(f) if f is not None else None, st),
+              "papc_weight_prologue_f32")
     return table
+
+
+class XyzL1Fin(ctypes.Structure):
+    _fields_ = [("gram_partial", ctypes.c_void_p), ("parts", ctypes.c_int32), ("M", ctypes.c_int64), ("w", ctypes.c_void_p), ("ldw", ctypes.c_int32),
+                ("xcol0", ctypes.c_int32), ("bias", ctypes.c_void_p), ("gamma", ctypes.c_void_p), ("beta", ctypes.c_void_p), ("eps", ctypes.c_float),
+                ("momentum", ctypes.c_float), ("C", ctypes.c_int32)] + [(k, ctypes.c_void_p) for k in
+                ("mean", "invstd", "scale", "shift", "running_mean", "running_var", "wf", "gram")]
+
+
+def l1_handover(table, w):
+    ent = table.get(("l1", w.data_ptr())) if table is not None else None
+    if ent is None or tuple(ent[0].shape) != (4, w.shape[0]) or tuple(ent[1].shape) != (w.shape[0], 4):
+        return None
+    return ent
+
+
+def planes_handover(table, key, shape):
+    ent = table.get(key) if table is not None else None
+    return ent[0] if ent is not None and tuple(ent[1]) == tuple(shape) else None
 
 
 def xyz_first_layer_ok(M, c1, c2, n_layers):
@@ -177,13 +235,18 @@
                     assert tuple(xc.shape) == (M, 4) and tuple(gpart.shape) == (1, 16)
                 else:
                     xc, gpart = xyz_pregroup(xyz, new_xyz, idx)
-                cst = torch.empty(4, cout, device=dev, dtype=torch.float32)
-                wf = torch.empty(cout, 4, device=dev, dtype=torch.float32)
-                gram = torch.empty(16, device=dev, dtype=torch.float64)
+                pre = l1_handover(spec.wt_table, w)
+                if pre is not None:
+                    cst, wf, gram = pre
+                else:
+                    cst = torch.empty(4, cout, device=dev, dtype=torch.float32)
+                    wf = torch.empty(cout, 4, device=dev, dtype=torch.float32)
+                    gram = torch.empty(16, device=dev, dtype=torch.float64)
                 rm, rv = (bn_buffers[l] if bn_buffers is not None else (None, None))
-                check(lib.papc_xyz_l1_finalize_f32(ptr(gpart), nparts, M, ptr(w2), cin, 0, ptr(b), ptr(gamma), ptr(beta), spec.eps, spec.momentum,
-                                                   cout, cst[0].data_ptr(), cst[1].data_ptr(), cst[2].data_ptr(), cst[3].data_ptr(), ptr(rm), ptr(rv),
-                                                   ptr(wf), ptr(gram), st), "papc_xyz_l1_finalize_f32")
+                if pre is None:
+                    check(lib.papc_xyz_l1_finalize_f32(ptr(gpart), nparts, M, ptr(w2), cin, 0, ptr(b), ptr(gamma), ptr(beta), spec.eps, spec.momentum,
+                                                       cout, cst[0].data_ptr(), cst[1].data_ptr(), cst[2].data_ptr(), cst[3].data_ptr(), ptr(rm), ptr(rv),
+                                                       ptr(wf), ptr(gram), st), "papc_xyz_l1_finalize_f32")
                 ys.append(None)
                 consts.append(cst)
                 prev_y, prev_sc, prev_sh = None, cst[2], cst[3]
diff --git a/papc_amd/models.py b/papc_amd/models.py
--- a/papc_amd/models.py
+++ b/papc_amd/models.py
@@ -103,9 +103,21 @@
             from . import smallm
             from .mlp import precompute_wt
             ws = [c.weight for c in list(self.sa1.mlp_convs)[1:]] + [c.weight for c in self.sa2.mlp_convs]
+            planes, l1 = [], None
             if not (smallm.takes_group_all(B, self.sa2.npoint, [c.weight.shape[0] for c in self.sa3.mlp_convs])):
                 ws += [c.weight for c in self.sa3.mlp_convs]
-            wt = precompute_wt(ws, feat_blocks=[(self.sa2.mlp_convs[0].weight, True)])
+            else:
+                D3 = self.sa3.mlp_convs[0].weight.shape[1] - 3
+                if D3 % 4 == 0:
+                    planes = [(c.weight, (D3, 3) if l == 0 else True) for l, c in enumerate(self.sa3.mlp_convs)]
+            if plan is not None and pl[0] is not None and norm is None and self.sa1._xyz_first(B):
+                from .plan import Level
+                pre = Level.parse(pl[0], B * self.sa1.npoint, [self.sa1.nsample]).xyz_pre
+                conv, bn = self.sa1.mlp_convs[0], self.sa1.mlp_bns[0]
+                if pre is not None and len(pre) == 2 and tuple(pre[1].shape) == (1, 16):
+                    l1 = (conv.weight, conv.bias, bn.weight, bn.bias, (bn.running_mean, bn.running_var), bn.eps, 0.9,
+                          B * self.sa1.npoint * self.sa1.nsample, pre[1])
+            wt = precompute_wt(ws, feat_blocks=[(self.sa2.mlp_convs[0].weight, True)], planes=planes, l1=l1)
         l1_xyz, l1_points = self.sa1(xyz, norm, s[0], sampled=pl[0], wt_table=wt)
         if after_sa1 is not None:
             after_sa1()
diff --git a/papc_amd/smallm.py b/papc_amd/smallm.py
--- a/papc_amd/smallm.py
+++ b/papc_amd/smallm.py
@@ -99,11 +99,23 @@
         fcol0 = (3 if spec.xyz_first else 0) if not plain else 0
         n_in = cin0 if plain else spec.D
 
+        from .mlp import planes_handover
+        wtab = getattr(spec, "wt_table", None)
+        given = []
+        for l in range(L):
+            rows, off = (ch[l], 0) if l > 0 else (n_in, fcol0)
+            given.append((planes_handover(wtab, ("p", params[4 * l].data_ptr()), (ch[l + 1], ch[l], 0)),
+                          planes_handover(wtab, ("pt", params[4 * l].data_ptr()), (rows, ch[l + 1], off)) if want_bwd and (l > 0 or in_grad) else None))
+        handed = all(g[0] is not None and (g[1] is not None or not (want_bwd and (l > 0 or in_grad))) for l, g in enumerate(given))
         w2s, wp, wtp, jobs = [], [], [None] * L, []
         for l in range(L):
             w2 = params[4 * l].reshape(ch[l + 1], ch[l])
             assert w2.is_contiguous()
             w2s.append(w2)
+            if handed:
+                wp.append(given[l][0])
+                wtp[l] = given[l][1]
+                continue
             wp.append(_planes(lib, ch[l + 1], ch[l], dev))
             jobs.append((w2.data_ptr(), ch[l], 1, ch[l + 1], ch[l], wp[l].data_ptr()))
             if want_bwd and (l > 0 or in_grad):
diff --git a/papc_amd/stack.py b/papc_amd/stack.py
--- a/papc_amd/stack.py
+++ b/papc_amd/stack.py
@@ -28,7 +28,8 @@
 class SaIo(ctypes.Structure):
     _fields_ = [("xyz", c_p), ("sb", c_l), ("sn", c_l), ("sc", c_l), ("new_xyz", c_p), ("feats", c_p), ("idx", c_p), ("x_rows", c_p),
                 ("xc", c_p), ("xc_gram", c_p), ("compact", ctypes.POINTER(CompactSrc)), ("consts3", c_p), ("consts3_ld", c_i),
-                ("layer", SaLayer * MAXL), ("out", c_p), ("saved", c_p), ("scratch", c_p), ("plists", c_p), ("wfeat", c_p)]
+                ("layer", SaLayer * MAXL), ("out", c_p), ("saved", c_p), ("scratch", c_p), ("plists", c_p), ("wfeat", c_p),
+                ("l1_cst", c_p), ("l1_wf", c_p), ("l1_gram", c_p), ("wplanes", c_p * MAXL), ("wtplanes", c_p * MAXL)]
 
 
 class SaPlan(ctypes.Structure):
@@ -103,6 +104,22 @@
         if ent is not None and ent[1] == bool(spec.xyz_first) and tuple(ent[0].shape) == (params[0].shape[0], cin0 - 3) and cin0 - 3 == spec.D:
             io.wfeat = ent[0].data_ptr()
             keep.append(ent[0])
+    if wtab is not None and L >= 1:
+        from .mlp import l1_handover, planes_handover
+        pre = l1_handover(wtab, params[0])
+        if pre is not None and feats is None and x_rows is None:
+            io.l1_cst, io.l1_wf, io.l1_gram = (t.data_ptr() for t in pre)
+            keep.extend(pre)
+        if x_rows is None and idx is None:
+            fcol0 = 3 if spec.xyz_first else 0
+            for l in range(L):
+                w = params[4 * l]
+                cout = w.shape[0]
+                cin = w.numel() // cout
+                t = planes_handover(wtab, ("p", w.data_ptr()), (cout, cin, 0))
+                tt = planes_handover(wtab, ("pt", w.data_ptr()), (cin, cout, 0) if l > 0 else (spec.D, cout, fcol0))
+                io.wplanes[l], io.wtplanes[l] = ptr(t), ptr(tt)
+                keep.extend([t, tt])
     c3 = _consts3(params[0].device)
     keep.append(c3)
     io.consts3, io.consts3_ld = c3.data_ptr(), c3.shape[1]
@@ -161,6 +178,8 @@
         ctx.nostore, ctx.xyz1, ctx.lin0, ctx.planes = bool(plan.nostore), bool(plan.xyz1), bool(plan.lin0), bool(plan.planes)
         ctx.bn_buffers = bn_buffers
         ctx.wt_table = spec.wt_table
+        from .mlp import l1_handover
+        ctx.l1_cst = l1_handover(spec.wt_table, params[0])[0] if io.l1_cst else None
         ctx.feats_needs_grad = feats is not None and feats.requires_grad and not spec.cut_gather_grad
         ctx.x_needs_grad = plain and x_rows.requires_grad
         ctx.save_for_backward(xyz, new_xyz, feats, idx, x_rows, *params)
@@ -176,6 +195,8 @@
         am = view(plan.off_argmax, G * cs[-1], torch.int32)
         ys = [None if plan.off_y[l] < 0 else view(plan.off_y[l], M * cs[l], torch.float32).view(M, cs[l]) for l in range(L)]
         cst = [view(plan.off_cst[l], 4 * cs[l], torch.float32).view(4, cs[l]) for l in range(L)]
+        if plan.xyz1 and getattr(ctx, "l1_cst", None) is not None:
+            cst[0] = ctx.l1_cst
         return (None if am is None else am.view(G, cs[-1])), ys, cst
 
     @staticmethod
```

Result: no change. 21510 (-0.1%).
